# AdvancedPhotonSource/tike

Hardware: AMD Instinct MI355X
Metric: diffraction patterns/sec/GPU (256x256, 8-mode probe) (higher is better)
Workload: dtype c64; 1 GPU; c3; positions_per_gpu=10000, modes=8, detector=256, eigen_probes=1, solver=lstsq_grad, num_batch=10, chunk_positions=1000, position_correction=False, object_update=after every minibatch (batch_method wobbly_center), route=no_farplane

## Files before the change

include/tike_amd.h:

```cpp
#ifndef TIKE_AMD_H
#define TIKE_AMD_H

#ifdef __cplusplus
extern "C" {
#endif

#define TIKE_ERR_ARG 1000001
#define TIKE_ERR_UNSUPPORTED 1000002
#define TIKE_ERR_COMM 2000000
#define TIKE_COMM_ID_BYTES 128

#define TIKE_ABI_VERSION 15

const char* tike_build_id(void);

int tike_abi_version(void);

int tike_set_deterministic(int on, void* scratch, long bytes);

int tike_init(void);

int tike_patch_fwd(const void* images, void* patches, const float* positions, int nimage, int H,
                   int W, int nscan, int nrepeat, int patch_width, int padded_width,
                   void* stream);
int tike_patch_adj(void* images, const void* patches, const float* positions, int nimage, int H,
                   int W, int nscan, int nrepeat, int patch_width, int padded_width, int npatch,
                   void* stream);

int tike_conv_fwd(const void* psi, const float* scan, const void* probe, int probe_per_scan,
                  void* nearplane, int nscan, int S, int pw, int det, int H, int W, void* stream);
int tike_conv_adj(const void* nearplane, const float* scan, const void* probe,
                  int probe_per_scan, void* psi, int nscan, int S, int pw, int det, int H, int W,
                  void* stream);
int tike_conv_adj_probe(const void* nearplane, const float* scan, const void* psi,
                        void* probe_adj, int nscan, int S, int pw, int det, int H, int W,
                        void* stream);

int tike_fft2(const void* in, void* out, long ntile, int n, int inverse, float scale,
              void* stream);

int tike_fft2_supported(int n);

int tike_fft2_general(const void* in, void* out, long ntile, int n, int inverse, float scale,
                      int lines_per_group_rows, int lines_per_group_cols, void* stream);

int tike_ptycho_fwd(const void* psi, const float* scan, const void* probe, int probe_per_scan,
                    const void* eigen_probe, const float* eigen_weights, int num_eigen,
                    int eigen_modes, void* farplane, int nscan, int S, int pw, int det, int H,
                    int W, float scale, int sub_batch, void* stream);

int tike_ptycho_adj(const void* farplane, const void* probe, int probe_per_scan,
                    const float* scan, const void* psi, void* psi_adj, void* probe_adj,
                    void* objproj_work, float* acc_work, int nscan, int S, int pw, int det,
                    int H, int W, float scale, int sub_batch, void* stream);

int tike_ptycho_fwd_intensity(const void* psi, const float* scan, const void* probe,
                              int probe_per_scan, const void* unique_probe,
                              const float* eigen_weights, int num_eigen, int eigen_modes,
                              void* farplane, float* intensity, void* patches, int nscan, int S,
                              int pw, int det, int H, int W, float scale, void* stream);

int tike_ptycho_fwd_intensity_only(const void* psi, const float* scan, const void* probe,
                                   int probe_per_scan, const void* unique_probe,
                                   const float* eigen_weights, int num_eigen, int eigen_modes,
                                   void* scratch, float* intensity, int nscan, int S, int pw,
                                   int det, int H, int W, float scale, void* stream);

int tike_ptycho_fwd_gradient_scale(const void* psi, const float* scan, const void* probe,
                                   int probe_per_scan, const void* unique_probe,
                                   const float* eigen_weights, int num_eigen, int eigen_modes,
                                   void* scratch, float* intensity, void* patches,
                                   const float* data, const unsigned char* measured,
                                   float* gscale, float* costs, int nscan, int S, int pw, int det,
                                   int H, int W, float scale, int model, float unmeasured_scaling,
                                   long num_measured, void* stream);

int tike_fwd_pass1(const void* psi, const float* scan, const void* probe, int probe_per_scan,
                   const void* unique_probe, const void* eigen_probe,
                   const float* eigen_weights, int num_eigen, int eigen_modes, void* scratch,
                   void* patches, int nscan, int S, int pw, int det, int H, int W, void* stream);
int tike_fwd_gradient_scale(const void* scratch, const void* data, int data_u16,
                            const unsigned char* measured, float* gscale, float* intensity,
                            float* costs, void* farplane, int nscan, int S, int det, float scale,
                            int model, float unmeasured_scaling, long num_measured,
                            void* stream);

int tike_grad_ifft2_crop(const void* colin, const float* gscale, const float* mode_scale,
                         const unsigned char* measured, int S, void* work, void* chi,
                         long ntile, int det, int pw, float fwd_scale, float inv_scale,
                         void* stream);

int tike_fwd_grad_ifft2_pass1(const void* scratch, const void* data, int data_u16,
                              const unsigned char* measured, float* costs, void* work,
                              int nscan, int S, int det, float fwd_scale, int model,
                              float unmeasured_scaling, long num_measured, void* stream);
// ... 224 lines not shown
                         float* esum, float* work, void* stream);
int tike_eigen_dsum(const float* sums, int B, long P, float* dsum, void* stream);
int tike_eigen_weights(const float* sums, int B, long P, const float* dsum, double count,
                       float* weights_c, long weights_row, void* coefs_c, int coef_stride,
                       const float* esum, void* stream);

int tike_cgrad_direction(const float* update_planar, const void* update_complex, void* gradient,
                         void* direction, long n, int first, const float* costs, int ncost,
                         double count, double* state, double* sums, void* stream);

int tike_cgrad_line_search(int variable, const void* x, const void* d, void* xs,
                           const void* other, const float* scan, const void* data,
                           int data_u16, void* scratch, float* costs, int nscan, int chunk,
                           int S, int det, int H, int W, float fwd_scale, double count,
                           double* state, int* skip, int nslots, void* stream);

int tike_cgrad_line_search_masked(int variable, const void* x, const void* d, void* xs,
                                  const void* other, const float* scan, const void* data,
                                  int data_u16, void* scratch, float* costs, int nscan, int chunk,
                                  int S, int det, int H, int W, float fwd_scale, double count,
                                  double* state, int* skip, int nslots,
                                  const unsigned char* measured, int model, long num_measured,
                                  void* stream);

int tike_cgrad_line_search_linear(int variable, const void* x, const void* d, void* xs,
                                  const void* other, const float* scan, const void* data,
                                  int data_u16, void* far_a, int a_valid, void* far_b,
                                  float* costs_k, int nscan, int chunk, int S, int det, int H,
                                  int W, float fwd_scale, double count, double* state,
                                  int stage, double* sums, void* stream);

int tike_cgrad_line_search_linear_masked(int variable, const void* x, const void* d, void* xs,
                                         const void* other, const float* scan, const void* data,
                                         int data_u16, void* far_a, int a_valid, void* far_b,
                                         float* costs_k, int nscan, int chunk, int S, int det,
                                         int H, int W, float fwd_scale, double count,
                                         double* state, int stage, double* sums,
                                         const unsigned char* measured, int model,
                                         long num_measured, void* stream);

int tike_eigen_pixel_update1(const void* patches, const void* chi0, const void* mpu0,
                             const void* eigen0, const float* eigen_proj,
                             const float* weights_c, long weights_row, const float* norm,
                             void* update, int nscan, int pw, int chi_modes, const float* stats,
                             const float* costs, float eps, float* sums3, const void* psi,
                             const float* scan, int H, int W, void* stream);
int tike_lstsq_tail_mid(void* eigen0, const void* update, int npix, float* nacc,
                        float beta_eigen, const float* stats, int B, float eps,
                        const float* sums3, double count, int recover_psi, int recover_probe,
                        float* tail3, void* stream);
int tike_eigen_position_sums1(const void* patches, const void* chi0, const void* mpu0,
                              const void* eigen0, float* sums5, float* dsum, int nscan, int pw,
                              int chi_modes, const void* psi, const float* scan, int H, int W,
                              void* stream);
int tike_lstsq_tail_finish(const float* tail3, const float* sums3, double count, float* steps,
                           void* probe, void* combined, const void* mpu, float inv_num_batch,
                           long nprobe, float* weights, long weights_row, int S, int m,
                           const float* stats, const float* sums5, int B, int npix,
                           void* stream);

int tike_ifft2_pass2_gradients_eproj(const void* work, const void* patches, const void* probe,
                                     const void* eigen_probe, const float* eigen_weights,
                                     int num_eigen, int eigen_modes, void* objproj, void* chi0,
                                     void* m_probe_update, float mpu_scale, int nscan, int S,
                                     int det, float inv_scale, float* qtab, float* q,
                                     void* stream);
int tike_eigen_pixel_update1q(const void* patches, const void* chi0, const void* mpu0,
                              const void* eigen0, const float* q, const float* weights_c,
                              long weights_row, const float* norm, void* update, int nscan,
                              int pw, int chi_modes, const void* psi, const float* scan, int H,
                              int W, float* c0part, float* eproj_out, void* stream);
int tike_lstsq_step_stats_eigen1(const void* chi, const float* scan,
                                 const void* object_update_precond, const void* probe,
                                 const void* eigen_probe, const float* eigen_weights,
                                 int eigen_modes, const void* m_probe_update, const void* patches,
                                 const void* update, float* nacc, double count, float beta_eigen,
                                 float* stats, float* sums5, int nscan, int S, int chi_modes,
                                 int pw, int H, int W, void* stream);
int tike_lstsq_tail_solve1(void* eigen0, const void* update, int npix, const float* nacc,
                           float beta_eigen, const float* stats, const float* costs,
                           const float* sums5, int B, float eps, double count, int recover_psi,
                           int recover_probe, float* sums3, float* tail3, void* stream);

int tike_lstsq_chunk_gradients(const void* psi, const float* scan, const void* probe,
                               const void* eigen_probe, const float* eigen_weights,
                               int num_eigen, int eigen_modes, const void* data, int data_u16,
                               const unsigned char* measured, int model,
                               float unmeasured_scaling, long num_measured, void* scratch,
                               void* work, float* gscale, void* patches, float* costs,
                               void* objproj, void* chi0, void* m_probe_update,
                               float mpu_scale, float* object_acc, int nscan, int S, int det,
                               int H, int W, float fwd_scale, float inv_scale, void* stream);

int tike_lstsq_chunk_gradients_positions(
    const void* psi, const float* scan, const void* probe, const void* eigen_probe,
    const float* eigen_weights, int num_eigen, int eigen_modes, const void* data, int data_u16,
    const unsigned char* measured, int model, float unmeasured_scaling, long num_measured,
    void* scratch, void* work, float* gscale, void* patches, float* costs, void* objproj,
    void* chi0, void* m_probe_update, float mpu_scale, float* object_acc, int nscan, int S,
    int det, int H, int W, float fwd_scale, float inv_scale, const float* taps, int taps_radius,
    float* intensity_work, float* numerator, float* denominator, void* stream);

int tike_comm_unique_id(void* id);
int tike_comm_create(const void* id, int nranks, int rank, void** comm);
int tike_comm_destroy(void* comm);
int tike_comm_allreduce_sum(void* comm, void* buf, long count, int f64, void* stream);
int tike_comm_broadcast(void* comm, void* buf, long nbytes, int root, void* stream);

int tike_cluster_farthest_fill(const float* points, long n, long* owner, int num_cluster,
                               long turns);
int tike_cluster_swap_sweep(const double* dist, long n, int k, long* label, const long* best,
                            const long* order, double* regret, int* moved);

#ifdef __cplusplus
}
#endif
#endif
```

tike_amd/_lib.py:

```python
import ctypes
import os
import re

import torch

_HERE = os.path.dirname(os.path.abspath(__file__))
LIB_PATH = os.environ.get("TIKE_AMD_LIB") or os.path.join(
    _HERE, "csrc", "libtike_amd.so")
HEADER_PATH = os.path.join(os.path.dirname(_HERE), "include", "tike_amd.h")

ABI_VERSION = 15
ERR_ARG = 1000001
ERR_UNSUPPORTED = 1000002
ERR_COMM = 2000000
COMM_ID_BYTES = 128

if not os.path.isfile(LIB_PATH):
    raise ImportError(
        f"{LIB_PATH} not found: build the HIP library first "
        "(`make -C tike_amd/csrc` or `python -c 'import __graft_entry__ as g; "
        "g.build()'`). tike_amd has no CPU fallback.")

lib = ctypes.CDLL(LIB_PATH)

_p = ctypes.c_void_p
_i = ctypes.c_int
_l = ctypes.c_long
_f = ctypes.c_float
_d = ctypes.c_double

_PROTOTYPES = {
    "tike_abi_version": [],
    "tike_init": [],
    "tike_set_deterministic": [_i, _p, _l],
    "tike_patch_fwd": [_p, _p, _p, _i, _i, _i, _i, _i, _i, _i, _p],
    "tike_patch_adj": [_p, _p, _p, _i, _i, _i, _i, _i, _i, _i, _i, _p],
    "tike_conv_fwd": [_p, _p, _p, _i, _p, _i, _i, _i, _i, _i, _i, _p],
    "tike_conv_adj": [_p, _p, _p, _i, _p, _i, _i, _i, _i, _i, _i, _p],
    "tike_conv_adj_probe": [_p, _p, _p, _p, _i, _i, _i, _i, _i, _i, _p],
    "tike_fft2": [_p, _p, _l, _i, _i, _f, _p],
    "tike_fft2_supported": [_i],
    "tike_fft2_general": [_p, _p, _l, _i, _i, _f, _i, _i, _p],
    "tike_pfa_supported": [_i, _i, _i],
    "tike_pfa_fwd_gather": [_p, _p, _p, _i, _p, _p, _p, _i, _i, _p, _p, _i, _i, _i,
                            _i, _i, _i, _p],
    "tike_pfa_fwd_subtiles_supported": [_i, _i, _i],
    "tike_pfa_fwd_subtiles": [_p, _p, _p, _p, _p, _i, _i, _p, _p, _p, _i, _i,
                              _i, _i, _i, _i, _p],
    "tike_pfa_fft2": [_p, _p, _l, _i, _i, _p],
    "tike_pfa_combine_gradient": [_p, _p, _p, _p, _i, _i, _i, _f, _i, _f, _l, _i,
                                  _p],
    "tike_pfa_inv_products": [_p, _p, _p, _i, _p, _p, _p, _i, _i, _p, _p, _p, _f,
                              _i, _i, _i, _i, _f, _p],
    "tike_gen_supported": [_i, _i, _i],
    "tike_gen_fwd_rows": [_p, _p, _p, _i, _p, _p, _p, _i, _i, _p, _p, _i, _i, _i,
                          _i, _i, _i, _p],
    "tike_gen_cols_gradient": [_p, _p, _p, _p, _p, _i, _i, _i, _i, _f, _i, _f,
                               _l, _p],
    "tike_gen_inv_rows_gradients": [_p, _p, _p, _i, _p, _p, _p, _i, _i, _p, _p,
                                    _p, _f, _i, _i, _i, _i, _f, _p],
    "tike_fresnel_spect_prop": [_p, _p, _p, _l, _i, _i, _f, _f, _p],
    "tike_fft2_pass1": [_p, _p, _l, _i, _i, _p],
    "tike_fft2_pass2_inplace": [_p, _l, _i, _i, _f, _p],
    "tike_slice_step": [_p, _p, _p, _p, _i, _i, _i, _i, _i, _f, _p],
    "tike_fft2_pass2_intensity": [_p, _p, _l, _i, _i, _i, _f, _i, _p],
    "tike_fresnel_colpass": [_p, _p, _i, _p, _l, _i, _f, _p],
    "tike_ifft2_pass2_products": [_p, _p, _p, _p, _i, _p, _p, _f, _p, _i, _i, _i,
                                  _i, _i, _i, _f, _p],
    "tike_ptycho_fwd": [_p, _p, _p, _i, _p, _p, _i, _i, _p, _i, _i, _i, _i,
                        _i, _i, _f, _i, _p],
    "tike_ptycho_adj": [_p, _p, _i, _p, _p, _p, _p, _p, _p, _i, _i, _i, _i, _i,
                        _i, _f, _i, _p],
    "tike_ifft2_crop": [_p, _p, _p, _l, _i, _i, _f, _p],
    "tike_ptycho_fwd_intensity": [_p, _p, _p, _i, _p, _p, _i, _i, _p, _p, _p,
                                  _i, _i, _i, _i, _i, _i, _f, _p],
    "tike_gradient_scale": [_p, _p, _p, _p, _p, _i, _i, _i, _f, _l, _p],
    "tike_ifft2_crop_scaled": [_p, _p, _i, _p, _p, _l, _i, _i, _f, _p],
    "tike_ifft2_crop_scaled_modes": [_p, _p, _p, _p, _i, _p, _p, _l, _i, _i, _f,
                                     _p],
    "tike_poisson_steps": [_p, _p, _p, _p, _p, _i, _i, _i, _f, _f, _i, _p],
    "tike_poisson_steps_handoff": [_p, _p, _i, _p, _p, _p, _p, _p, _i, _i, _i, _f,
                                   _f, _l, _f, _f, _p],
    "tike_scale_modes": [_p, _p, _p, _l, _i, _p],
    "tike_ptycho_fwd_intensity_only": [_p, _p, _p, _i, _p, _p, _i, _i, _p, _p,
                                       _i, _i, _i, _i, _i, _i, _f, _p],
    "tike_ptycho_fwd_gradient_scale": [_p, _p, _p, _i, _p, _p, _i, _i, _p, _p,
                                       _p, _p, _p, _p, _p, _i, _i, _i, _i, _i,
                                       _i, _f, _i, _f, _l, _p],
    "tike_fwd_pass1": [_p, _p, _p, _i, _p, _p, _p, _i, _i, _p, _p, _i, _i, _i,
                       _i, _i, _i, _p],
    "tike_fwd_gradient_scale": [_p, _p, _i, _p, _p, _p, _p, _p, _i, _i, _i, _f,
                                _i, _f, _l, _p],
    "tike_grad_ifft2_pass1": [_p, _p, _p, _p, _i, _p, _l, _i, _f, _p],
    "tike_fwd_grad_ifft2_pass1": [_p, _p, _i, _p, _p, _p, _i, _i, _i, _f, _i, _f,
                                  _l, _p],
    "tike_fwd_grad_ifft2_pass1_slices": [_p, _p, _i, _p, _p, _p, _i, _i, _i, _f, _i, _f,
                                  _l, _p, _i, _p],
    "tike_ifft2_pass1_scaled": [_p, _p, _p, _p, _i, _p, _l, _i, _p],
    "tike_ifft2_pass2_gradients": [_p, _p, _p, _p, _p, _i, _i, _p, _p, _p, _f,
                                   _i, _i, _i, _f, _p],
    "tike_ifft2_pass2_gradients_scaled": [_p, _p, _p, _p, _p, _i, _i, _p, _p,
                                          _p, _f, _i, _i, _i, _f, _p, _p],
    "tike_ifft2_pass2_eigen_fits": [_i, _i, _i],
    "tike_ifft2_pass2_gradients_modes": [_p, _p, _p, _p, _p, _i, _i, _p, _p,
                                         _p, _f, _i, _i, _i, _f, _i, _i, _i, _p],
    "tike_poisson_steps_grad_ifft2_pass1": [_p, _p, _i, _p, _p, _p, _p, _p, _i,
                                            _i, _i, _f, _f, _l, _f, _f, _p],
    "tike_object_update_precond": [_p, _p, _p, _f, _p, _p, _p, _l, _p],
    "tike_lstsq_step_sums": [_p, _p, _i, _f, _p, _p],
    "tike_lstsq_step_solve": [_p, _i, _f, _p, _d, _i, _i, _p, _p],
    "tike_probe_update": [_p, _p, _p, _p, _f, _l, _p],
    "tike_eigen_weights0": [_p, _p, _i, _i, _i, _i, _p, _p],
    "tike_eigen_proj_mean": [_p, _i, _p, _l, _p, _l, _i, _p, _p],
    "tike_eigen_normalise": [_p, _p, _d, _f, _i, _p, _p, _p],
    "tike_eigen_dsum": [_p, _i, _l, _p, _p],
    "tike_eigen_weights": [_p, _i, _l, _p, _d, _p, _l, _p, _i, _p, _p],
    "tike_grad_ifft2_crop": [_p, _p, _p, _p, _i, _p, _p, _l, _i, _i, _f, _f,
                             _p],
    "tike_position_sums": [_p, _p, _i, _p, _p, _p, _i, _i, _p, _i, _p, _p, _i,
                           _i, _i, _p],
    "tike_rpie_position_sums": [_p, _p, _p, _p, _i, _p, _p, _i, _i, _p, _i, _p,
                                _p, _p, _i, _i, _i, _i, _i, _p],
    "tike_farplane_gradient": [_p, _p, _p, _p, _p, _i, _i, _i, _i, _i, _f, _l,
                               _p],
    "tike_intensity": [_p, _p, _l, _i, _l, _p],
    "tike_cost_each_pattern": [_p, _p, _p, _l, _l, _i, _p],
    "tike_objective_grad": [_p, _p, _p, _p, _l, _i, _l, _i, _p],
    "tike_lstsq_gradients": [_p, _p, _p, _p, _p, _p, _i, _i, _p, _p, _p, _p, _i,
                             _i, _i, _i, _i, _p],
    "tike_varying_probe": [_p, _p, _p, _i, _i, _p, _i, _i, _i, _p],
    "tike_scatter_patches": [_p, _p, _p, _i, _i, _i, _i, _p],
    "tike_eigen_position_sums": [_p, _p, _p, _p, _p, _i, _i, _i, _p, _i, _i,
                                 _i, _p],
    "tike_eigen_pixel_update": [_p, _p, _p, _p, _p, _i, _i, _i, _p, _p, _i, _i,
                                _i, _p],
    "tike_probe_grad": [_p, _p, _p, _p, _p, _i, _i, _i, _i, _i, _p],
    "tike_probe_preconditioner": [_p, _p, _p, _i, _i, _i, _i, _p],
    "tike_psi_preconditioner": [_p, _p, _p, _i, _i, _i, _i, _p],
    "tike_scatter_amplitudes": [_p, _p, _p, _i, _i, _i, _i, _p],
    "tike_lstsq_step_stats": [_p, _p, _p, _p, _p, _p, _p, _i, _i, _p, _p, _p,
                              _p, _i, _i, _i, _i, _i, _i, _p, _p, _p],
    "tike_eigen_pixel_update1": [_p, _p, _p, _p, _p, _p, _l, _p, _p, _i, _i, _i,
                                 _p, _p, _f, _p, _p, _p, _i, _i, _p],
    "tike_lstsq_tail_mid": [_p, _p, _i, _p, _f, _p, _i, _f, _p, _d, _i, _i, _p,
                            _p],
    "tike_eigen_position_sums1": [_p, _p, _p, _p, _p, _p, _i, _i, _i, _p, _p,
                                  _i, _i, _p],
    "tike_lstsq_tail_finish": [_p, _p, _d, _p, _p, _p, _p, _f, _l, _p, _l, _i,
                               _i, _p, _p, _i, _i, _p],
    "tike_ifft2_pass2_gradients_eproj": [_p, _p, _p, _p, _p, _i, _i, _p, _p,
                                         _p, _f, _i, _i, _i, _f, _p, _p, _p],
    "tike_eigen_pixel_update1q": [_p, _p, _p, _p, _p, _p, _l, _p, _p, _i, _i,
                                  _i, _p, _p, _i, _i, _p, _p, _p],
    "tike_lstsq_step_stats_eigen1": [_p, _p, _p, _p, _p, _p, _i, _p, _p, _p,
                                     _p, _d, _f, _p, _p, _i, _i, _i, _i, _i,
                                     _i, _p],
    "tike_lstsq_tail_solve1": [_p, _p, _i, _p, _f, _p, _p, _p, _i, _f, _d, _i,
                               _i, _p, _p, _p],
    "tike_lstsq_chunk_gradients": [_p, _p, _p, _p, _p, _i, _i, _p, _i, _p, _i,
                                   _f, _l, _p, _p, _p, _p, _p, _p, _p, _p, _f,
                                   _p, _i, _i, _i, _i, _i, _f, _f, _p],
    "tike_lstsq_chunk_gradients_positions": [
        _p, _p, _p, _p, _p, _i, _i, _p, _i, _p, _i, _f, _l, _p, _p, _p, _p, _p,
        _p, _p, _p, _f, _p, _i, _i, _i, _i, _i, _f, _f, _p, _i, _p, _p, _p, _p],
    "tike_cgrad_direction": [_p, _p, _p, _p, _l, _i, _p, _i, _d, _p, _p, _p],
    "tike_cgrad_line_search": [_i, _p, _p, _p, _p, _p, _p, _i, _p, _p, _i, _i,
                               _i, _i, _i, _i, _f, _d, _p, _p, _i, _p],
    "tike_cgrad_line_search_linear": [_i, _p, _p, _p, _p, _p, _p, _i, _p, _i, _p,
                                      _p, _i, _i, _i, _i, _i, _i, _f, _d, _p, _i,
                                      _p, _p],
    "tike_cgrad_line_search_masked": [_i, _p, _p, _p, _p, _p, _p, _i, _p, _p,
                                      _i, _i, _i, _i, _i, _i, _f, _d, _p, _p,
                                      _i, _p, _i, _l, _p],
    "tike_cgrad_line_search_linear_masked": [_i, _p, _p, _p, _p, _p, _p, _i, _p,
                                             _i, _p, _p, _i, _i, _i, _i, _i, _i,
                                             _f, _d, _p, _i, _p, _p, _i, _l, _p],
    "tike_comm_unique_id": [_p],
    "tike_comm_create": [_p, _i, _i, ctypes.POINTER(_p)],
    "tike_comm_destroy": [_p],
    "tike_comm_allreduce_sum": [_p, _p, _l, _i, _p],
    "tike_comm_broadcast": [_p, _p, _l, _i, _p],
    "tike_cluster_farthest_fill": [_p, _l, _p, _i, _l],
    "tike_cluster_swap_sweep": [_p, _l, _i, _p, _p, _p, _p, _p],
}


def build_id():
    try:
        fn = lib.tike_build_id
    except AttributeError:
        return ""
    fn.restype = ctypes.c_char_p
    fn.argtypes = []
    return fn().decode()


def declared_symbols():
    with open(HEADER_PATH) as f:
        text = f.read()
    return sorted(set(re.findall(r"^int\s+(tike_\w+)\s*\(", text, flags=re.M)))


for _name, _args in _PROTOTYPES.items():
    try:
        _fn = getattr(lib, _name)
    except AttributeError as e:
        raise ImportError(
            f"{LIB_PATH} does not export {_name}: it was built from another "
            "include/tike_amd.h; rebuild it (`make -C tike_amd/csrc`).") from e
    _fn.argtypes = _args
    _fn.restype = ctypes.c_int


def _check_abi_version():
    got = lib.tike_abi_version()
    m = re.search(r"^#define\s+TIKE_ABI_VERSION\s+(\d+)", open(HEADER_PATH).read(),
                  flags=re.M) if os.path.isfile(HEADER_PATH) else None
    if got != ABI_VERSION or (m and int(m.group(1)) != ABI_VERSION):
        raise ImportError(
            f"{LIB_PATH} reports ABI version {got}, include/tike_amd.h "
            f"{m.group(1) if m else '?'}, this binding expects {ABI_VERSION}: "
            "rebuild the library (`make -C tike_amd/csrc`).")


_check_abi_version()


def check(rc, what=""):
    if rc == 0:
        return
    if rc == ERR_ARG:
        raise ValueError(f"{what}: incompatible shapes / arguments")
    if rc == ERR_UNSUPPORTED:
        raise ValueError(f"{what}: unsupported size for the HIP path")
    if rc >= ERR_COMM:
        raise RuntimeError(f"{what}: RCCL error {rc - ERR_COMM}")
    raise RuntimeError(f"{what}: HIP error {rc}")


DETERMINISTIC = os.environ.get("TIKE_DETERMINISTIC", "0") == "1"
DETERMINISTIC_SCRATCH_MIB = int(os.environ.get("TIKE_DETERMINISTIC_MIB", "256"))
# ... 19 lines not shown
```

tike_amd/_tuning.py:

```python
import os


def _flag(name, default):
    return os.environ.get(name, "1" if default else "0") == "1"


def _int(name, default=None):
    v = os.environ.get(name)
    return int(v) if v else default


one_launch_512 = _flag("TIKE_ONE_LAUNCH_512", True)
poisson_steps_in_pass2 = _flag("TIKE_POISSON_LINEAR", True)
chunk_positions = _int("TIKE_CHUNK_POSITIONS")
eigen_sums_gather = _flag("TIKE_EIGEN_SUMS_GATHER", True)
stats_gather = _flag("TIKE_STATS_GATHER", False)
fused_tail = _flag("TIKE_FUSED_TAIL", True)
precond_chunk = _int("TIKE_PRECOND_CHUNK", 512)
multislice_slice_step = _flag("TIKE_MS_SLICE_STEP", True)
multislice_first_stored = _flag("TIKE_MS_FIRST_STORED", True)
multislice_step_back = _flag("TIKE_MS_STEP_BACK", True)
cgrad_graphs = _flag("TIKE_CGRAD_GRAPHS", False)
fwd_sub_mib = (float(os.environ["TIKE_FWD_SUB_MIB"])
               if os.environ.get("TIKE_FWD_SUB_MIB") else None)
```

tike_amd/csrc/internal.h:

```cpp
#pragma once
#include "common.h"

int tk_fft2(const cf* in, cf* out, long ntile, int n, int inverse, float scale,
            hipStream_t stream);
int tk_fft2_general(const cf* in, cf* out, long ntile, int n, int inverse, float scale,
                    int l_rows, int l_cols, hipStream_t stream);
int tk_conv_fwd(const cf* psi, const float* scan, const TkProbe& probe, cf* nearplane, int nscan,
                int S, int pw, int det, int H, int W, hipStream_t stream);
int tk_conv_adj(const cf* nearplane, const float* scan, const TkProbe& probe, cf* psi, int nscan,
                int S, int pw, int det, int H, int W, hipStream_t stream);
int tk_conv_adj_probe(const cf* nearplane, const float* scan, const cf* psi, cf* probe_adj,
                      int nscan, int S, int pw, int det, int H, int W, hipStream_t stream);

int tk_fft2_pass1(const cf* in, cf* out, long ntile, int det, bool inverse, bool keep,
                  hipStream_t stream);
int tk_ifft2_pass2_products(cf* work, const cf* psi, const float* scan, const cf* probe,
                            int probe_per_scan, cf* objproj, float* pnum, float pnum_scale,
                            cf* chi0, int out, int nscan, int S, int det, int H, int W,
                            float inv_scale, hipStream_t stream);

bool tk_deterministic();
float* tk_det_scratch(size_t bytes);

struct TkCostSink {
  float* costs;
  float* part;
  int nslots;
};
#if defined(__HIPCC__)
__device__ __forceinline__ void tk_cost_add(const TkCostSink& k, long n, int slot, float v) {
  if (k.part != nullptr)
    k.part[n * k.nslots + slot] = v;
  else
    unsafeAtomicAdd(&k.costs[n], v);
}
#endif
int tk_cost_sink(float* costs, long nscan, int nslots, hipStream_t stream, TkCostSink* sink);
int tk_cost_finish(const TkCostSink& sink, long nscan, hipStream_t stream);
int tk_ordered_sum(float* out, const float* part, long n, int nparts, bool accumulate,
                   hipStream_t stream, int out_stride = 1);
```

tike_amd/csrc/lstsq.hip:

```cpp
#include "fft_engine2.h"
#include <type_traits>

#include "internal.h"
#include "tike_amd.h"

#ifndef TK_STATS_PAIRS
#define TK_STATS_PAIRS 1
#endif
static const bool g_stats_pairs = TK_STATS_PAIRS != 0;

constexpr int TK_STRIP = 32;
#define TK_ATOMIC_ADD(p, v) unsafeAtomicAdd(p, v)

template <bool REAL_ONLY, class ValueFn, class Sink>
__device__ __forceinline__ void scatter_footprint_rows(ValueFn&& value, float fx, float fy,
                                                       int pw, int r0, int r1, Sink&& sink) {
  for (int x0 = 0; x0 < pw; x0 += blockDim.x) {
    const int xp = x0 + threadIdx.x;
    const bool active = xp < pw;
    cf uprev = mk(0.f, 0.f), uprev_last = mk(0.f, 0.f);
    constexpr int RG = 4;
    cf vv[RG], ll[RG], nv[RG], nl[RG];
    auto load_group = [&](int yb, cf (&a)[RG], cf (&b)[RG]) {
      const int xpc = active ? xp : pw - 1;
// ... 726 lines not shown
#pragma unroll
            for (int i = 0; i < 8; ++i) {
              cf t = (pc[i] * u[g + i]) * w0;
              if (REDUCE) {
                slot[(g + i) * 64] = m == 0 ? t : slot[(g + i) * 64] + t;
              } else {
                if (eig) {
#pragma unroll 1
                  for (int c = 0; c < nE; ++c)
                    t = t + (eigl[((c * probe.Sm + s) * RB + g + i) * (64 * CW) + cw * 64 + lane] *
                             u[g + i]) * wn[(c + 1) * probe.S + s];
                }
                tk_st_stream(tk_at(objproj + (long)n * P + slice0 + (g + i) * ROW, lo), t);
              }
            }
            if (!HOIST) __builtin_amdgcn_sched_barrier(0);
          }
          if (REDUCE && eig) {
#pragma unroll 1
            for (int c = 0; c < nE; ++c) {
              const float wc = wn[(c + 1) * probe.S + s];
              const cf* __restrict__ el =
                  eigl + ((c * probe.Sm + s) * RB) * (64 * CW) + cw * 64 + lane;
              if (QN && c == 0 && s == 0) {
                float q = 0.f;
#pragma unroll
                for (int yb = 0; yb < RB; ++yb) {
                  const cf e = el[yb * (64 * CW)];
                  slot[yb * 64] = slot[yb * 64] + (e * u[yb]) * wc;
                  const cf t = conjf(O[yb]) * u[yb];
                  q += t.x * e.x - t.y * e.y;
                }
                q_store(q, n);
                continue;
              }
#pragma unroll
              for (int yb = 0; yb < RB; ++yb)
                slot[yb * 64] = slot[yb * 64] + (el[yb * (64 * CW)] * u[yb]) * wc;
            }
          }
        }
      } else if (REDUCE && m == 0) {
#pragma unroll
        for (int yb = 0; yb < RB; ++yb) slot[yb * 64] = mk(0.f, 0.f);
      }
    }
    if (REDUCE) {
      __syncthreads();
#pragma unroll
      for (int q = 0; q < RB / MW; ++q) {
        const int yb = mw + MW * q;
        cf sum = slots[yb * 64];
#pragma unroll
        for (int k = 1; k < MW; ++k) sum = sum + slots[(k * RB + yb) * 64];
        if (accumulate) sum = sum + *tk_at(objproj + (long)n * P + slice0 + yb * ROW, lo);
        tk_st_stream(tk_at(objproj + (long)n * P + slice0 + yb * ROW, lo), sum);
      }
      if (NBUF == 1) __syncthreads();
    }
  }
  if (mpu != nullptr) {
#pragma unroll
    for (int m = 0; m < MPW; ++m) {
      const int s = mw + MW * m;
      if (s < S) {
#pragma unroll
        for (int yb = 0; yb < RB; ++yb) {
          if (mpu_part != nullptr) {
            const long ci = (nchunk_ - 1) - b0 / chunk;
            float* o = tk_at(mpu_part + 2 * ((ci * S + s) * P + slice0 + yb * ROW), lb);
            o[0] = acc[m][yb].x * mpu_scale;
            o[1] = acc[m][yb].y * mpu_scale;
          } else {
            float* o = tk_at(mpu + 2 * ((long)s * P + slice0 + yb * ROW), lb);
            unsafeAtomicAdd(o, acc[m][yb].x * mpu_scale);
            unsafeAtomicAdd(o + 1, acc[m][yb].y * mpu_scale);
          }
        }
      }
    }
  }
}

__global__ __launch_bounds__(256) void pass2_q_finish_kernel(const float* __restrict__ qtab,
                                                             int slots, int nscan,
                                                             float* __restrict__ q) {
  const int n = blockIdx.x * 4 + (int)(threadIdx.x >> 6), k = threadIdx.x & 63;
  if (n >= nscan) return;
  float a = k < slots ? qtab[(long)k * nscan + n] : 0.f;
  a = tk_wave_sum(a);
  if (k == 0) q[n] = a;
}

template <int N, int MW_, int MPW_>
static bool launch_pass2_qn(dim3 grid, size_t lds, hipStream_t stream, const cf* work,
                            const cf* patches, const TkProbe& pr, cf* objproj, cf* chi0,
                            float* mpu, float mpu_scale, int nscan, int S, float inv_scale,
                            int chunk, float* mpu_part, const float* mode_scale, float* qtab) {
  if constexpr (N <= 256) {
    hipLaunchKernelGGL((ifft2_pass2_gradients_kernel<N, MW_, MPW_, true, true, false, true>),
                       grid, dim3(256), lds, stream, work, patches, pr, objproj, chi0, mpu,
                       mpu_scale, nscan, S, inv_scale, chunk, mpu_part, mode_scale, 0, 0, qtab);
    return true;
  } else {
    return false;
  }
}

static int launch_pass2_gradients(const void* work, const void* patches, const void* probe,
                                  const void* eigen_probe, const float* eigen_weights,
                                  int num_eigen, int eigen_modes, void* objproj, void* chi0,
                                  void* m_probe_update, float mpu_scale, int nscan, int S,
                                  int det, float inv_scale, const float* mode_scale,
                                  hipStream_t stream, int Stot = 0, int accumulate = 0,
                                  float* qtab = nullptr, float* q = nullptr) {
  TK_CHECK_ARG(nscan >= 0 && S >= 1 && det >= 1);
  if (nscan == 0) return TK_OK;
  TK_CHECK_ARG(work && patches && (probe || !objproj));
  if (S > 8 || (det != 128 && det != 256 && det != 512)) return TK_ERR_UNSUPPORTED;
  const bool qn = q != nullptr;
  TK_CHECK_ARG(!qn || qtab);
  if (qn && (Stot != 0 || det > 256 || !objproj || !eigen_probe || !eigen_weights ||
             num_eigen < 1 || eigen_modes < 1))
    return TK_ERR_UNSUPPORTED;
  const bool grp = Stot != 0;
  if (grp && objproj && S < 2) return TK_ERR_UNSUPPORTED;
  const TkProbe pr = tk_make_probe(probe, 0, eigen_probe, eigen_weights, num_eigen, eigen_modes,
                                   grp ? Stot : S, det);
  int MW = S >= 3 ? 4 : S;
  if (det == 128 && MW == 1) MW = 2;
  auto eig_bytes = [&](int mw) {
    return sizeof(cf) * (size_t)num_eigen * eigen_modes * (det / 16) * 64 * (4 / mw);
  };
  if (objproj && eigen_weights && eigen_probe)
    while (MW < 4 && eig_bytes(MW) > 32 * 1024) MW *= 2;
  const int MPW = S > 4 ? 2 : 1;
  const int nslice = 16 * (det / (64 * (4 / MW)));
  int nchunk = (1024 + nslice - 1) / nslice;
  {
    int unit = 512, a = nslice;
    while (a % 2 == 0 && unit > 1) { a /= 2; unit /= 2; }
    if (nchunk >= unit) nchunk = nchunk / unit * unit;
  }
  int chunk = (nscan + nchunk - 1) / nchunk;
  if (chunk < 8) chunk = 8;
  nchunk = (nscan + chunk - 1) / chunk;
  const dim3 grid((unsigned)(nslice * nchunk)), block(256);
  float* mpu_part = nullptr;
  const long mpu_len = 2L * S * det * det;
  if (m_probe_update && tk_deterministic()) {
    mpu_part = tk_det_scratch(sizeof(float) * (size_t)mpu_len * nchunk);
    if (mpu_part == nullptr) return TK_ERR_ARG;
  }
  size_t eig_lds = 0;
  if (objproj && eigen_weights && eigen_probe) eig_lds = eig_bytes(MW);
  if (eig_lds > 32 * 1024) return TK_ERR_UNSUPPORTED;
#define TK_P2G(N, MW_, MPW_)                                                                 \
  do {                                                                                       \
    if (qn) {                                                                                \
      if (!launch_pass2_qn<N, MW_, MPW_>(grid, eig_lds, stream, (const cf*)work,             \
                                         (const cf*)patches, pr, (cf*)objproj, (cf*)chi0,    \
                                         (float*)m_probe_update, mpu_scale, nscan, S,        \
                                         inv_scale, chunk, mpu_part, mode_scale, qtab))      \
        return TK_ERR_UNSUPPORTED;                                                           \
    } else if (grp && !objproj)                                                              \
      hipLaunchKernelGGL((ifft2_pass2_gradients_kernel<N, MW_, MPW_, false, true, true>),    \
                         grid, block, 0,                                                     \
                         stream, (const cf*)work, (const cf*)patches, pr, (cf*)objproj,      \
                         (cf*)chi0, (float*)m_probe_update, mpu_scale, nscan, S, inv_scale,  \
                         chunk, mpu_part, mode_scale, Stot, accumulate);                     \
    else if (grp && eig_lds > 0)                                                             \
      hipLaunchKernelGGL((ifft2_pass2_gradients_kernel<N, MW_, MPW_, true, true, true>),     \
                         grid, block, eig_lds,                                               \
                         stream, (const cf*)work, (const cf*)patches, pr, (cf*)objproj,      \
                         (cf*)chi0, (float*)m_probe_update, mpu_scale, nscan, S, inv_scale,  \
                         chunk, mpu_part, mode_scale, Stot, accumulate);                     \
    else if (grp)                                                                            \
      hipLaunchKernelGGL((ifft2_pass2_gradients_kernel<N, MW_, MPW_, true, false, true>),    \
                         grid, block, 0,                                                     \
                         stream, (const cf*)work, (const cf*)patches, pr, (cf*)objproj,      \
                         (cf*)chi0, (float*)m_probe_update, mpu_scale, nscan, S, inv_scale,  \
                         chunk, mpu_part, mode_scale, Stot, accumulate);                     \
    else if (objproj && eig_lds > 0)                                                         \
      hipLaunchKernelGGL((ifft2_pass2_gradients_kernel<N, MW_, MPW_, true>), grid, block,    \
                         eig_lds,                                                            \
                         stream, (const cf*)work, (const cf*)patches, pr, (cf*)objproj,      \
                         (cf*)chi0, (float*)m_probe_update, mpu_scale, nscan, S, inv_scale,  \
                         chunk, mpu_part, mode_scale);                                       \
    else if (objproj)                                                                        \
      hipLaunchKernelGGL((ifft2_pass2_gradients_kernel<N, MW_, MPW_, true, false>), grid,    \
                         block, 0,                                                           \
                         stream, (const cf*)work, (const cf*)patches, pr, (cf*)objproj,      \
                         (cf*)chi0, (float*)m_probe_update, mpu_scale, nscan, S, inv_scale,  \
                         chunk, mpu_part, mode_scale);                                       \
    else                                                                                     \
      hipLaunchKernelGGL((ifft2_pass2_gradients_kernel<N, MW_, MPW_, false>), grid, block,   \
                         0, stream, (const cf*)work, (const cf*)patches, pr, (cf*)objproj,   \
                         (cf*)chi0, (float*)m_probe_update, mpu_scale, nscan, S, inv_scale,  \
                         chunk, mpu_part, mode_scale);                                       \
  } while (0)
#define TK_P2G_N(N)                     \
  do {                                  \
    if (MW == 1)                        \
      TK_P2G(N < 256 ? 256 : N, 1, 1);  \
    else if (MW == 2)                   \
      TK_P2G(N, 2, 1);                  \
    else if (MPW == 1)                  \
      TK_P2G(N, 4, 1);                  \
    else                                \
      TK_P2G(N, 4, 2);                  \
  } while (0)
  switch (det) {
    case 128: TK_P2G_N(128); break;
    case 256: TK_P2G_N(256); break;
    default: TK_P2G_N(512); break;
  }
#undef TK_P2G_N
#undef TK_P2G
  TK_LAUNCH_CHECK();
  if (qn) {
    hipLaunchKernelGGL(pass2_q_finish_kernel, dim3((nscan + 3) / 4), dim3(256), 0, stream,
                       qtab, det / 4, nscan, q);
    TK_LAUNCH_CHECK();
  }
  if (mpu_part != nullptr)
    return tk_ordered_sum((float*)m_probe_update, mpu_part, mpu_len, nchunk, true, stream);
  return TK_OK;
}

extern "C" int tike_ifft2_pass2_gradients(const void* work, const void* patches,
                                          const void* probe, const void* eigen_probe,
                                          const float* eigen_weights, int num_eigen,
                                          int eigen_modes, void* objproj, void* chi0,
                                          void* m_probe_update, float mpu_scale, int nscan,
                                          int S, int det, float inv_scale, void* stream) {
  TK_ENTER();
  return launch_pass2_gradients(work, patches, probe, eigen_probe, eigen_weights, num_eigen,
                                eigen_modes, objproj, chi0, m_probe_update, mpu_scale, nscan, S,
                                det, inv_scale, nullptr, (hipStream_t)stream);
}

extern "C" int tike_ifft2_pass2_gradients_scaled(const void* work, const void* patches,
                                                 const void* probe, const void* eigen_probe,
                                                 const float* eigen_weights, int num_eigen,
                                                 int eigen_modes, void* objproj, void* chi0,
                                                 void* m_probe_update, float mpu_scale,
                                                 int nscan, int S, int det, float inv_scale,
                                                 const float* mode_scale, void* stream) {
  TK_ENTER();
  TK_CHECK_ARG(nscan == 0 || mode_scale != nullptr);
  return launch_pass2_gradients(work, patches, probe, eigen_probe, eigen_weights, num_eigen,
                                eigen_modes, objproj, chi0, m_probe_update, mpu_scale, nscan, S,
                                det, inv_scale, mode_scale, (hipStream_t)stream);
}

extern "C" int tike_ifft2_pass2_gradients_eproj(const void* work, const void* patches,
                                                const void* probe, const void* eigen_probe,
                                                const float* eigen_weights, int num_eigen,
                                                int eigen_modes, void* objproj, void* chi0,
                                                void* m_probe_update, float mpu_scale,
                                                int nscan, int S, int det, float inv_scale,
                                                float* qtab, float* q, void* stream) {
  TK_ENTER();
  TK_CHECK_ARG(nscan == 0 || (qtab && q));
  return launch_pass2_gradients(work, patches, probe, eigen_probe, eigen_weights, num_eigen,
                                eigen_modes, objproj, chi0, m_probe_update, mpu_scale, nscan, S,
                                det, inv_scale, nullptr, (hipStream_t)stream, 0, 0, qtab, q);
}

extern "C" int tike_ifft2_pass2_eigen_fits(int det, int num_eigen, int eigen_modes) {
  if (det < 16 || num_eigen < 0 || eigen_modes < 0) return 0;
  return sizeof(cf) * (size_t)num_eigen * eigen_modes * (det / 16) * 64 <= 32 * 1024 ? 1 : 0;
}

extern "C" int tike_ifft2_pass2_gradients_modes(const void* work, const void* patches,
                                                const void* probe, const void* eigen_probe,
                                                const float* eigen_weights, int num_eigen,
                                                int eigen_modes, void* objproj, void* chi0,
                                                void* m_probe_update, float mpu_scale,
                                                int nscan, int S, int det, float inv_scale,
                                                int mode0, int nmodes, int accumulate,
                                                void* stream) {
  TK_ENTER();
  TK_CHECK_ARG(S >= 1 && det >= 1 && mode0 >= 0 && nmodes >= 1 && mode0 + nmodes <= S);
  TK_CHECK_ARG(nscan == 0 || (work && (probe || !objproj)));
  const long P = (long)det * det;
  const bool first = mode0 == 0;
  if (first ? eigen_modes > nmodes : false) return TK_ERR_UNSUPPORTED;
  return launch_pass2_gradients(
      (const cf*)work + mode0 * P, patches, probe ? (const cf*)probe + mode0 * P : nullptr,
      first ? eigen_probe : nullptr, eigen_weights ? eigen_weights + mode0 : nullptr,
      first ? num_eigen : (eigen_weights ? num_eigen : 0), first ? eigen_modes : 0, objproj,
      first ? chi0 : nullptr,
      m_probe_update ? (void*)((float*)m_probe_update + 2 * mode0 * P) : nullptr, mpu_scale,
      nscan, nmodes, det, inv_scale, nullptr, (hipStream_t)stream, S, accumulate);
}

template <int RW>
__global__ __launch_bounds__(256) void probe_precond_rows_kernel(
    const float* __restrict__ scan, const cf* __restrict__ psi, float* __restrict__ out,
    int nscan, int pw, int H, int W, int chunk, float* __restrict__ part) {
  typedef float tk_v4f __attribute__((ext_vector_type(4)));
  const long P = (long)pw * pw;
  const long total = (long)H * W;
  const int cols = pw < 256 ? pw : 256, ncb = pw / cols;
  const int x = ((int)blockIdx.x % ncb) * cols + (int)threadIdx.x % cols;
  const int y0 = (((int)blockIdx.x / ncb) * (256 / cols) + (int)threadIdx.x / cols) * RW;
  const int b0 = blockIdx.y * chunk;
  const int b1 = min(nscan, b0 + chunk);
  float acc[RW];
#pragma unroll
  for (int r = 0; r < RW; ++r) acc[r] = 0.f;
  bool inside = true;
  for (int b = b0; b < b1; ++b) {
    const TkCorner c = tk_corner(scan, b);
    inside = inside && c.sy >= 0 && c.sx >= 0 && c.sy + pw < H && c.sx + pw < W;
  }
  if (inside) {
    const unsigned row_bytes = (unsigned)W * (unsigned)sizeof(cf);
    const unsigned lane_off = (unsigned)y0 * row_bytes + (unsigned)x * (unsigned)sizeof(cf);
#pragma unroll 2
    for (int b = b0; b < b1; ++b) {
      const TkCorner c = tk_corner(scan, b);
      const unsigned off = (unsigned)(c.sy * W + c.sx) * (unsigned)sizeof(cf) + lane_off;
      tk_v4f t[RW + 1];
#pragma unroll
      for (int r = 0; r <= RW; ++r)
        __builtin_memcpy(&t[r], reinterpret_cast<const char*>(psi) + off + (unsigned)r * row_bytes,
                         sizeof(tk_v4f));
#pragma unroll
      for (int r = 0; r < RW; ++r) {
        cf o = mk(t[r].x * c.w00, t[r].y * c.w00);
        o.x += t[r].z * c.w01;
        o.y += t[r].w * c.w01;
        o.x += t[r + 1].x * c.w10;
        o.y += t[r + 1].y * c.w10;
        o.x += t[r + 1].z * c.w11;
        o.y += t[r + 1].w * c.w11;
        acc[r] += norm2(o);
      }
    }
  } else {
    for (int b = b0; b < b1; ++b) {
      const TkCorner c = tk_corner(scan, b);
#pragma unroll
      for (int r = 0; r < RW; ++r) {
        const int y = c.sy + y0 + r, xx = c.sx + x;
// ... 457 lines not shown
  __device__ __forceinline__ cf at(long n, long p) const {
    cf r = conjf(patches[n * P + p]) * chi0[n * XS + p] - mpu0[p];
    if (!C0)
      for (int k = 0; k < c; ++k) r = r - coefs[n * C + k] * eigen[((long)k * Sm) * P + p];
    return r;
  }
};

template <bool C0>
__global__ __launch_bounds__(256) void eigen_position_sums_kernel(const TkResidual R,
                                                                  float* __restrict__ sums,
                                                                  int nscan) {
  __shared__ float red[4];
  const cf* __restrict__ E = R.eigen + ((long)R.c * R.Sm) * R.P;
  for (int n = blockIdx.x; n < nscan; n += gridDim.x) {
    float a[5] = {0.f, 0.f, 0.f, 0.f, 0.f};
    for (long p = threadIdx.x; p < R.P; p += blockDim.x) {
      const cf e = E[p];
      const cf r = R.at<C0>(n, p);
      const cf phi = R.patches[n * R.P + p] * e;
      const cf x = R.chi0[n * R.XS + p];
      a[0] += r.x * e.x + r.y * e.y;
      a[1] += x.x * phi.x + x.y * phi.y;
      a[2] += norm2(phi);
      const cf re = r * conjf(e);
      a[3] += re.x;
      a[4] += re.y;
    }
#pragma unroll
    for (int k = 0; k < 5; ++k) {
      const float v = tk_block_sum256(a[k], red);
      if (threadIdx.x == 0) sums[(long)n * 5 + k] = v;
    }
  }
}

template <bool C0>
__global__ __launch_bounds__(256) void eigen_pixel_update_kernel(const TkResidual R,
                                                                 const float* __restrict__ pm,
                                                                 float* __restrict__ update,
                                                                 int nscan, int chunk,
                                                                 float* __restrict__ part) {
  const long p = (long)blockIdx.x * blockDim.x + threadIdx.x;
  if (p >= R.P) return;
  const int b0 = blockIdx.y * chunk;
  const int b1 = min(nscan, b0 + chunk);
  cf acc = mk(0.f, 0.f);
#pragma unroll 4
  for (int n = b0; n < b1; ++n) {
    const cf r = R.at<C0>(n, p);
    const float w = pm[n];
    acc.x += r.x * w;
    acc.y += r.y * w;
  }
  if (part != nullptr) {
    part[2 * ((long)blockIdx.y * R.P + p)] = acc.x;
    part[2 * ((long)blockIdx.y * R.P + p) + 1] = acc.y;
    return;
  }
  unsafeAtomicAdd(&update[2 * p], acc.x);
  unsafeAtomicAdd(&update[2 * p + 1], acc.y);
}

__device__ __forceinline__ cf tk_patch_pixel(const cf* __restrict__ psi, unsigned off,
                                             unsigned row_bytes, const TkCorner& c) {
  typedef float tk_v4f __attribute__((ext_vector_type(4)));
  tk_v4f u, l;
  __builtin_memcpy(&u, reinterpret_cast<const char*>(psi) + off, sizeof(u));
  __builtin_memcpy(&l, reinterpret_cast<const char*>(psi) + off + row_bytes, sizeof(l));
  cf o = mk(u.x * c.w00, u.y * c.w00);
  o.x += u.z * c.w01;
  o.y += u.w * c.w01;
  o.x += l.x * c.w10;
  o.y += l.y * c.w10;
  o.x += l.z * c.w11;
  o.y += l.w * c.w11;
  return o;
}
__device__ __forceinline__ bool tk_interior(const TkCorner& c, int pw, int H, int W) {
  return c.sy >= 0 && c.sx >= 0 && c.sy + pw < H && c.sx + pw < W && (long)H * W < (1L << 28);
}

constexpr int TK_C0_PARTS = 64;
__global__ __launch_bounds__(256) void eigen_proj_offset_kernel(const cf* __restrict__ mpu0,
                                                                const cf* __restrict__ E,
                                                                long P,
                                                                float* __restrict__ part) {
  __shared__ float red[4];
  float a = 0.f;
  for (long p = blockIdx.x * 256L + threadIdx.x; p < P; p += 256L * TK_C0_PARTS) {
    const cf m = mpu0[p], e = E[p];
    a += m.x * e.x + m.y * e.y;
  }
  a = tk_block_sum256(a, red);
  if (threadIdx.x == 0) part[blockIdx.x] = a;
}

__global__ __launch_bounds__(256) void eigen_pixel_update1_kernel(
    const TkResidual R, const float* __restrict__ eproj, const float* __restrict__ weights_c,
    long row, const float* __restrict__ norm, float inv_P, float* __restrict__ update, int nscan,
    int chunk, const float* __restrict__ stats, const float* __restrict__ costs, float eps,
    float* __restrict__ sums3, const cf* __restrict__ psi, const float* __restrict__ scan, int pw,
    int H, int W, float* __restrict__ part, const float* __restrict__ c0part,
    float* __restrict__ eproj_out) {
  float c0 = 0.f;
  if (c0part != nullptr) {
    for (int b = 0; b < TK_C0_PARTS; ++b) c0 += c0part[b];
  }
  if (blockIdx.x + 1 == gridDim.x) {
    if (blockIdx.y != 0) return;
    if (eproj_out != nullptr) {
      for (int n = threadIdx.x; n < nscan; n += 256) eproj_out[n] = eproj[n] - c0;
    }
    if (sums3 == nullptr) return;
    __shared__ float red[4];
    float a1 = 0.f, a4 = 0.f, c = 0.f;
    for (int n = threadIdx.x; n < nscan; n += 256) {
      a1 += stats[8 * n] + eps;
      a4 += stats[8 * n + 1] + eps;
      c += costs[n];
    }
    a1 = tk_block_sum256(a1, red);
    a4 = tk_block_sum256(a4, red);
    c = tk_block_sum256(c, red);
    if (threadIdx.x == 0) {
      sums3[0] = a1;
      sums3[1] = a4;
      sums3[2] = c;
    }
    return;
  }
  const long p = (long)blockIdx.x * blockDim.x + threadIdx.x;
  if (p >= R.P) return;
  const int b0 = blockIdx.y * chunk;
  const int b1 = min(nscan, b0 + chunk);
  const float inv_norm = 1.0f / norm[0];
  cf acc = mk(0.f, 0.f);
  bool gather = psi != nullptr;
  if (gather) {
    for (int n = b0; n < b1; ++n) gather = gather && tk_interior(tk_corner(scan, n), pw, H, W);
  }
  if (gather) {
    const int py = (int)(p / pw), px = (int)(p % pw);
    const unsigned row_bytes = (unsigned)W * (unsigned)sizeof(cf);
    const unsigned lane_off = (unsigned)py * row_bytes + (unsigned)px * (unsigned)sizeof(cf);
    const cf m0 = R.mpu0[p];
#pragma unroll 4
    for (int n = b0; n < b1; ++n) {
      const TkCorner c = tk_corner(scan, n);
      const cf x = R.chi0[n * R.XS + p];
      const cf o = tk_patch_pixel(
          psi, (unsigned)(c.sy * W + c.sx) * (unsigned)sizeof(cf) + lane_off, row_bytes, c);
      const cf r = conjf(o) * x - m0;
      const float w = ((eproj[n] - c0) * inv_P + weights_c[n * row]) * inv_norm;
      acc.x += r.x * w;
      acc.y += r.y * w;
    }
  } else {
#pragma unroll 4
    for (int n = b0; n < b1; ++n) {
      const cf r = R.at<true>(n, p);
      const float w = ((eproj[n] - c0) * inv_P + weights_c[n * row]) * inv_norm;
      acc.x += r.x * w;
      acc.y += r.y * w;
    }
  }
  if (part != nullptr) {
    part[2 * ((long)blockIdx.y * R.P + p)] = acc.x;
    part[2 * ((long)blockIdx.y * R.P + p) + 1] = acc.y;
    return;
  }
  unsafeAtomicAdd(&update[2 * p], acc.x);
  unsafeAtomicAdd(&update[2 * p + 1], acc.y);
}

__global__ __launch_bounds__(256) void column_sum_ordered_kernel(const float* __restrict__ table,
                                                                 int stride, int col, int n,
                                                                 float scale,
// ... 235 lines not shown
    const cf* __restrict__ chi_a = chi + ((long)n0 * chi_modes) * P;
    const cf* __restrict__ chi_b = chi + ((long)(n0 + 1) * chi_modes) * P;
    const cf* __restrict__ pat_a = patches + (long)n0 * P;
    const cf* __restrict__ pat_b = pat_a + P;
    auto tap = [](const tk_v4f u, const tk_v4f l, const TkCorner& c) {
      cf g = mk(u.x * c.w00, u.y * c.w00);
      g.x += u.z * c.w01;
      g.y += u.w * c.w01;
      g.x += l.x * c.w10;
      g.y += l.y * c.w10;
      g.x += l.z * c.w11;
      g.y += l.w * c.w11;
      return g;
    };
    auto sums = [](float* acc, const cf g, const cf o, const cf x0, const cf p0, const cf pn,
                   const cf m0) {
      const cf dOP = g * pn;
      const cf dPO = m0 * o;
      const cf OP = o * p0;
      acc[0] += norm2(dOP);
      acc[1] += norm2(dPO);
      const cf a2 = dOP * conjf(dPO);
      acc[2] += a2.x;
      acc[3] += a2.y;
      acc[4] += dOP.x * x0.x + dOP.y * x0.y;
      acc[5] += dPO.x * x0.x + dPO.y * x0.y;
      acc[6] += OP.x * x0.x + OP.y * x0.y;
      acc[7] += norm2(OP);
    };
    auto pixel = [&](const int p, const tk_v4f u0, const tk_v4f l0, const tk_v4f u1,
                     const tk_v4f l1) {
      const cf oa = pat_a[p], ob = pat_b[p];
      const cf xa = chi_a[p], xb = chi_b[p];
      const cf p0 = probe.probe[p];
      const cf m0 = mpu[p];
      const cf e1 = probe.eigen[p];
      const cf en = enew(e1, p);
      cf pa = p0 * s0, pb = p0 * s1;
      pa.x += t0 * e1.x;
      pa.y += t0 * e1.y;
      pb.x += t1 * e1.x;
      pb.y += t1 * e1.y;
      sums(a, tap(u0, l0, c0), oa, xa, p0, pa, m0);
      sums(b, tap(u1, l1, c1), ob, xb, p0, pb, m0);
      esum(ea, oa, xa, en, m0);
      esum(eb, ob, xb, en, m0);
    };
    auto taps16 = [&](const unsigned off) {
      tk_v4f t;
      __builtin_memcpy(&t, reinterpret_cast<const char*>(gobj) + off, sizeof(t));
      return t;
    };
    const int cols = pw < 256 ? pw : 256, groups = 256 / cols;
    const int rows = pw / (nsplit * groups);
    const int ybeg = (part * groups + (int)threadIdx.x / cols) * rows;
    for (int x = (int)threadIdx.x % cols; x < pw; x += 256) {
      unsigned rel = (unsigned)(ybeg * W + x);
      tk_v4f u0 = taps16((base0 + rel) * 8u), u1 = taps16((base1 + rel) * 8u);
      int p = ybeg * pw + x;
#pragma unroll 2
      for (int y = 0; y < rows; ++y) {
        rel += (unsigned)W;
        const tk_v4f l0 = taps16((base0 + rel) * 8u), l1 = taps16((base1 + rel) * 8u);
        pixel(p, u0, l0, u1, l1);
        u0 = l0;
        u1 = l1;
        p += pw;
      }
    }
#pragma unroll
    for (int k = 0; k < 8; ++k) {
      const float ta = tk_block_sum256(a[k], red);
      const float tb = tk_block_sum256(b[k], red);
      if (threadIdx.x == 0) {
        put(&stats[(long)n0 * 8 + k], ta);
        put(&stats[(long)n0 * 8 + 8 + k], tb);
      }
    }
    finish5(ea, n0);
    finish5(eb, n0 + 1);
  }
}

__global__ __launch_bounds__(256) void eigen_norm_sums1_kernel(const cf* __restrict__ E,
                                                               const cf* __restrict__ update,
                                                               int npix, float* __restrict__ nacc,
                                                               float* __restrict__ part) {
  __shared__ float red[4];
  float uu = 0.f, ee = 0.f, eu = 0.f;
  for (int i = blockIdx.x * 256 + threadIdx.x; i < npix; i += gridDim.x * 256) {
    const cf e = E[i], u = update[i];
    uu += norm2(u);
    ee += norm2(e);
    eu += e.x * u.x + e.y * u.y;
  }
  uu = tk_block_sum256(uu, red);
  ee = tk_block_sum256(ee, red);
  eu = tk_block_sum256(eu, red);
  if (threadIdx.x == 0) {
    if (part != nullptr) {
      part[3 * blockIdx.x] = uu;
      part[3 * blockIdx.x + 1] = ee;
      part[3 * blockIdx.x + 2] = eu;
    } else {
      unsafeAtomicAdd(&nacc[0], uu);
      unsafeAtomicAdd(&nacc[1], ee);
      unsafeAtomicAdd(&nacc[2], eu);
    }
  }
}

extern "C" int tike_lstsq_step_stats_eigen1(const void* chi, const float* scan,
                                            const void* object_update_precond, const void* probe,
                                            const void* eigen_probe, const float* eigen_weights,
                                            int eigen_modes, const void* m_probe_update,
                                            const void* patches, const void* update, float* nacc,
                                            double count, float beta_eigen, float* stats,
                                            float* sums5, int nscan, int S, int chi_modes,
                                            int pw, int H, int W, void* stream) {
  TK_ENTER();
  TK_CHECK_ARG(nscan >= 0 && S >= 1 && chi_modes >= 1 && pw >= 1 && H >= 1 && W >= 1 &&
               eigen_modes >= 1 && count > 0);
  TK_CHECK_ARG(probe && eigen_probe && eigen_weights && m_probe_update && update && nacc);
  const long P = (long)pw * pw;
  const long nitem = (nscan + 1) / 2;
  int nsplit = 1;
  while (nsplit < 16 && nitem * nsplit * 2 <= 8192 && P % (2048L * nsplit) == 0) nsplit *= 2;
  if (tk_deterministic()) nsplit = 1;
  const int groups = 256 / (pw < 256 ? pw : 256);
  if (!((pw % 256 == 0 || 256 % pw == 0) && pw % (nsplit * groups) == 0 &&
        (long)H * W < (1L << 28)))
    return TK_ERR_UNSUPPORTED;
  int grid = P >= 256 * 64 ? 64 : (int)((P + 255) / 256);
  float* part = nullptr;
  if (tk_deterministic()) {
    part = tk_det_scratch(sizeof(float) * 3 * (size_t)grid);
    if (part == nullptr) grid = 1;
  }
  hipLaunchKernelGGL(eigen_norm_sums1_kernel, dim3(grid), dim3(256), 0, (hipStream_t)stream,
                     (const cf*)eigen_probe, (const cf*)update, (int)P, nacc, part);
  TK_LAUNCH_CHECK();
  if (part != nullptr) {
    int rc = tk_ordered_sum(nacc, part, 3, grid, true, (hipStream_t)stream);
    if (rc) return rc;
  }
  if (nscan == 0) return TK_OK;
  TK_CHECK_ARG(chi && scan && object_update_precond && patches && stats && sums5);
  const TkProbe pr = tk_make_probe(probe, 0, eigen_probe, eigen_weights, 1, eigen_modes, S, pw,
                                   nullptr);
  if (nsplit > 1) {
    hipError_t e = hipMemsetAsync(stats, 0, sizeof(float) * 8 * (size_t)nscan, (hipStream_t)stream);
    if (e == hipSuccess)
      e = hipMemsetAsync(sums5, 0, sizeof(float) * 5 * (size_t)nscan, (hipStream_t)stream);
    if (e != hipSuccess) return (int)e;
  }
  hipLaunchKernelGGL(step_stats_eigen_pair_kernel, dim3(tk_grid(nitem * nsplit, 16)), dim3(256),
                     0, (hipStream_t)stream, (const cf*)chi, scan,
                     (const cf*)object_update_precond, pr, (const cf*)m_probe_update,
                     (const cf*)patches, (const cf*)update, (const float*)nacc,
                     (float)(1.0 / count), beta_eigen, stats, sums5, nscan, chi_modes, pw, H, W,
                     nsplit);
  TK_LAUNCH_CHECK();
  return TK_OK;
}

static TkResidual make_residual(const void* patches, const void* chi0, const void* mpu0,
                                const void* eigen, const void* coefs, int C, int Sm, int c,
                                int pw, int chi_modes) {
  TkResidual R;
  R.patches = (const cf*)patches;
  R.chi0 = (const cf*)chi0;
  R.mpu0 = (const cf*)mpu0;
  R.eigen = (const cf*)eigen;
  R.coefs = (const cf*)coefs;
  R.C = C;
  R.Sm = Sm;
  R.c = c;
  R.P = (long)pw * pw;
  R.XS = R.P * chi_modes;
  return R;
}

extern "C" int tike_eigen_position_sums(const void* patches, const void* chi0, const void* mpu0,
                                        const void* eigen_probe, const void* coefs,
                                        int num_eigen, int eigen_modes, int c, float* sums,
                                        int nscan, int pw, int chi_modes, void* stream) {
  TK_ENTER();
  TK_CHECK_ARG(nscan >= 0 && pw >= 1 && num_eigen >= 1 && c >= 0 && c < num_eigen &&
               chi_modes >= 1);
  if (nscan == 0) return TK_OK;
  TK_CHECK_ARG(patches && chi0 && mpu0 && eigen_probe && sums && (c == 0 || coefs));
  const TkResidual R = make_residual(patches, chi0, mpu0, eigen_probe, coefs, num_eigen,
                                     eigen_modes, c, pw, chi_modes);
  if (c == 0)
    hipLaunchKernelGGL(eigen_position_sums_kernel<true>, dim3(tk_grid(nscan, 16)), dim3(256), 0,
                       (hipStream_t)stream, R, sums, nscan);
  else
    hipLaunchKernelGGL(eigen_position_sums_kernel<false>, dim3(tk_grid(nscan, 16)), dim3(256),
                       0, (hipStream_t)stream, R, sums, nscan);
  TK_LAUNCH_CHECK();
  return TK_OK;
}

extern "C" int tike_eigen_pixel_update(const void* patches, const void* chi0, const void* mpu0,
                                       const void* eigen_probe, const void* coefs,
                                       int num_eigen, int eigen_modes, int c, const float* pm,
                                       void* update, int nscan, int pw, int chi_modes,
                                       void* stream) {
  TK_ENTER();
  TK_CHECK_ARG(nscan >= 0 && pw >= 1 && num_eigen >= 1 && c >= 0 && c < num_eigen &&
               chi_modes >= 1);
  if (nscan == 0) return TK_OK;
  TK_CHECK_ARG(patches && chi0 && mpu0 && eigen_probe && pm && update && (c == 0 || coefs));
  const long P = (long)pw * pw;
  float* part = nullptr;
  const int chunk = probe_chunk(nscan, 2 * P, &part);
  dim3 grid((unsigned)((P + 255) / 256), (unsigned)((nscan + chunk - 1) / chunk));
  const TkResidual R = make_residual(patches, chi0, mpu0, eigen_probe, coefs, num_eigen,
                                     eigen_modes, c, pw, chi_modes);
  if (c == 0)
    hipLaunchKernelGGL(eigen_pixel_update_kernel<true>, grid, dim3(256), 0, (hipStream_t)stream,
                       R, pm, (float*)update, nscan, chunk, part);
  else
    hipLaunchKernelGGL(eigen_pixel_update_kernel<false>, grid, dim3(256), 0,
                       (hipStream_t)stream, R, pm, (float*)update, nscan, chunk, part);
  TK_LAUNCH_CHECK();
  if (part != nullptr)
    return tk_ordered_sum((float*)update, part, 2 * P, (int)grid.y, true, (hipStream_t)stream);
  return TK_OK;
}

extern "C" int tike_eigen_pixel_update1(const void* patches, const void* chi0,
                                        const void* mpu0, const void* eigen0,
                                        const float* eigen_proj, const float* weights_c,
                                        long weights_row, const float* norm, void* update,
                                        int nscan, int pw, int chi_modes, const float* stats,
                                        const float* costs, float eps, float* sums3,
                                        const void* psi, const float* scan, int H, int W,
                                        void* stream) {
  TK_ENTER();
  TK_CHECK_ARG(nscan >= 0 && pw >= 1 && chi_modes >= 1 && weights_row >= 1);
  if (nscan == 0) {
    if (sums3) return (int)hipMemsetAsync(sums3, 0, 3 * sizeof(float), (hipStream_t)stream);
    return TK_OK;
  }
  TK_CHECK_ARG(!sums3 || (stats && costs));
  TK_CHECK_ARG(!psi || (scan && H >= 1 && W >= 1));
  TK_CHECK_ARG(patches && chi0 && mpu0 && eigen0 && eigen_proj && weights_c && norm && update);
  const long P = (long)pw * pw;
  float* part = nullptr;
  const int chunk = probe_chunk(nscan, 2 * P, &part);
  dim3 grid((unsigned)((P + 255) / 256) + 1, (unsigned)((nscan + chunk - 1) / chunk));
  const TkResidual R = make_residual(patches, chi0, mpu0, eigen0, nullptr, 1, 1, 0, pw, chi_modes);
  hipLaunchKernelGGL(eigen_pixel_update1_kernel, grid, dim3(256), 0, (hipStream_t)stream, R,
                     eigen_proj, weights_c, weights_row, norm, 1.0f / (float)P, (float*)update,
                     nscan, chunk, stats, costs, eps, sums3, (const cf*)psi, scan, pw, H, W,
                     part, nullptr, nullptr);
  TK_LAUNCH_CHECK();
  if (part != nullptr)
    return tk_ordered_sum((float*)update, part, 2 * P, (int)grid.y, true, (hipStream_t)stream);
  return TK_OK;
}

extern "C" int tike_eigen_pixel_update1q(const void* patches, const void* chi0,
                                         const void* mpu0, const void* eigen0, const float* q,
                                         const float* weights_c, long weights_row,
                                         const float* norm, void* update, int nscan, int pw,
                                         int chi_modes, const void* psi, const float* scan,
                                         int H, int W, float* c0part, float* eproj_out,
                                         void* stream) {
  TK_ENTER();
  TK_CHECK_ARG(nscan >= 0 && pw >= 1 && chi_modes >= 1 && weights_row >= 1);
  if (nscan == 0) return TK_OK;
  TK_CHECK_ARG(!psi || (scan && H >= 1 && W >= 1));
  TK_CHECK_ARG(patches && chi0 && mpu0 && eigen0 && q && weights_c && norm && update && c0part);
  const long P = (long)pw * pw;
  hipLaunchKernelGGL(eigen_proj_offset_kernel, dim3(TK_C0_PARTS), dim3(256), 0,
                     (hipStream_t)stream, (const cf*)mpu0, (const cf*)eigen0, P, c0part);
  float* part = nullptr;
  const int chunk = probe_chunk(nscan, 2 * P, &part);
  dim3 grid((unsigned)((P + 255) / 256) + 1, (unsigned)((nscan + chunk - 1) / chunk));
  const TkResidual R = make_residual(patches, chi0, mpu0, eigen0, nullptr, 1, 1, 0, pw, chi_modes);
  hipLaunchKernelGGL(eigen_pixel_update1_kernel, grid, dim3(256), 0, (hipStream_t)stream, R, q,
                     weights_c, weights_row, norm, 1.0f / (float)P, (float*)update, nscan, chunk,
                     nullptr, nullptr, 0.f, nullptr, (const cf*)psi, scan, pw, H, W, part,
                     c0part, eproj_out);
  TK_LAUNCH_CHECK();
  if (part != nullptr)
    return tk_ordered_sum((float*)update, part, 2 * P, (int)grid.y, true, (hipStream_t)stream);
  return TK_OK;
}

extern "C" int tike_eigen_position_sums1(const void* patches, const void* chi0,
                                         const void* mpu0, const void* eigen0, float* sums,
                                         float* dsum, int nscan, int pw, int chi_modes,
                                         const void* psi, const float* scan, int H, int W,
                                         void* stream) {
  TK_ENTER();
  TK_CHECK_ARG(nscan >= 0 && pw >= 1 && chi_modes >= 1);
  if (nscan == 0) return TK_OK;
  TK_CHECK_ARG(!psi || (scan && H >= 1 && W >= 1));
  TK_CHECK_ARG(patches && chi0 && mpu0 && eigen0 && sums && dsum);
  const TkResidual R = make_residual(patches, chi0, mpu0, eigen0, nullptr, 1, 1, 0, pw, chi_modes);
  const bool det = tk_deterministic();
  const int cols = pw < 256 ? pw : 256;
  const bool pairs = g_stats_pairs && psi != nullptr && nscan > 1 &&
                     (pw % 256 == 0 || 256 % pw == 0) && pw % (512 / cols) == 0 &&
                     (long)H * W < (1L << 28);
  if (pairs)
    hipLaunchKernelGGL(eigen_position_sums1_pair_kernel, dim3(tk_grid((nscan + 1) / 2, 16)),
                       dim3(512), 0, (hipStream_t)stream, R, sums, det ? nullptr : dsum, nscan,
                       (const cf*)psi, scan, pw, H, W);
  else
    hipLaunchKernelGGL(eigen_position_sums1_kernel, dim3(tk_grid(nscan, 16)), dim3(256), 0,
                       (hipStream_t)stream, R, sums, det ? nullptr : dsum, nscan, (const cf*)psi,
                       scan, pw, H, W);
  if (det)
    hipLaunchKernelGGL(column_sum_ordered_kernel, dim3(1), dim3(256), 0, (hipStream_t)stream, sums,
                       5, 2, nscan, 1.0f / (float)((long)pw * pw), dsum);
  TK_LAUNCH_CHECK();
  return TK_OK;
}

__global__ __launch_bounds__(256) void varying_probe_kernel(const TkProbe probe,
                                                            cf* __restrict__ out, long total,
                                                            long PP) {
  for (long i = blockIdx.x * (long)blockDim.x + threadIdx.x; i < total;
       i += (long)gridDim.x * blockDim.x) {
    const long pix = i % PP;
    const long ns = i / PP;
    out[i] = probe.at(ns / probe.Sm, (int)(ns % probe.Sm), pix);
  }
}

extern "C" int tike_varying_probe(const void* probe, const void* eigen_probe,
                                  const float* eigen_weights, int num_eigen, int eigen_modes,
                                  void* out, int nscan, int S, int pw, void* stream) {
  TK_ENTER();
  TK_CHECK_ARG(nscan >= 0 && S >= 1 && pw >= 1 && eigen_modes >= 1 && eigen_modes <= S);
  if (nscan == 0) return TK_OK;
  TK_CHECK_ARG(probe && eigen_weights && out && (num_eigen == 0 || eigen_probe));
  const long PP = (long)pw * pw;
  const long total = (long)nscan * eigen_modes * PP;
  hipLaunchKernelGGL(varying_probe_kernel, dim3(tk_grid((total + 255) / 256, 16)), dim3(256), 0,
                     (hipStream_t)stream,
                     tk_make_probe(probe, 0, eigen_probe, eigen_weights, num_eigen, eigen_modes,
                                   S, pw),
                     (cf*)out, total, PP);
  TK_LAUNCH_CHECK();
  return TK_OK;
}

struct TkTaps {
  float t[9];
  int r;
};

template <int RT>
__global__ __launch_bounds__(256) void position_sums_kernel(
    const cf* __restrict__ patches, const cf* __restrict__ chi, int chi_modes,
    const TkProbe probe, const TkTaps taps, float* __restrict__ num, float* __restrict__ den,
// ... 461 lines not shown
```

tike_amd/csrc/solver.hip:

```cpp
#include "internal.h"
#include "tike_amd.h"

__global__ __launch_bounds__(256) void object_update_precond_kernel(
    const float* __restrict__ acc, const cf* __restrict__ precond,
    const float* __restrict__ pmax, float alpha, cf* __restrict__ upd_sum,
    cf* __restrict__ upd_precond, float* __restrict__ combined, long npix) {
  const float am = alpha * pmax[0];
  for (long i = blockIdx.x * 256L + threadIdx.x; i < npix; i += gridDim.x * 256L) {
    const float re = acc[i], im = acc[npix + i];
    const float p = (1.0f - alpha) * precond[i].x;
    const float inv = 1.0f / sqrtf(p * p + am * am);
    if (upd_sum) upd_sum[i] = mk(re, im);
    if (upd_precond) upd_precond[i] = mk(re * inv, im * inv);
    if (combined) {
      combined[i] += re;
      combined[npix + i] += im;
    }
  }
}

extern "C" int tike_object_update_precond(const float* acc, const void* precond,
                                          const float* pmax, float alpha, void* upd_sum,
                                          void* upd_precond, float* combined, long npix,
                                          void* stream) {
  TK_ENTER();
  TK_CHECK_ARG(npix >= 0);
  if (npix == 0) return TK_OK;
  TK_CHECK_ARG(acc && precond && pmax);
  hipLaunchKernelGGL(object_update_precond_kernel, dim3(tk_grid((npix + 255) / 256, 8)),
                     dim3(256), 0, (hipStream_t)stream, acc, (const cf*)precond, pmax, alpha,
                     (cf*)upd_sum, (cf*)upd_precond, combined, npix);
  TK_LAUNCH_CHECK();
  return TK_OK;
}

__global__ __launch_bounds__(256) void step_sums_kernel(const float* __restrict__ stats,
                                                        const float* __restrict__ costs, int B,
                                                        float eps, float* __restrict__ sums) {
  __shared__ float red[4];
  float a1 = 0.f, a4 = 0.f, c = 0.f;
  for (int n = threadIdx.x; n < B; n += 256) {
    a1 += stats[8 * n] + eps;
    a4 += stats[8 * n + 1] + eps;
    if (costs) c += costs[n];
  }
  a1 = tk_block_sum256(a1, red);
  a4 = tk_block_sum256(a4, red);
  c = tk_block_sum256(c, red);
  if (threadIdx.x == 0) {
    sums[0] = a1;
    sums[1] = a4;
    sums[2] = c;
  }
}

__global__ __launch_bounds__(256) void step_solve_kernel(const float* __restrict__ stats, int B,
                                                         float eps,
                                                         const float* __restrict__ sums,
                                                         float inv_count, int recover_psi,
                                                         int recover_probe,
                                                         float* __restrict__ out) {
  __shared__ float red[4];
  const float r1 = 0.5f * sums[0] * inv_count, r4 = 0.5f * sums[1] * inv_count;
  float so = 0.f, sp = 0.f;
  for (int n = threadIdx.x; n < B; n += 256) {
    const float* s = stats + 8 * n;
    const float A1 = s[0] + eps + r1, A4 = s[1] + eps + r4;
    const float b1 = s[4], b2 = s[5];
    float x1 = 0.f, x2 = 0.f;
    if (recover_psi && recover_probe) {
      const float det = A1 * A4 - (s[2] * s[2] + s[3] * s[3]);
      x1 = -(s[2] * b2 - A4 * b1) / det;
      x2 = (A1 * b2 - s[2] * b1) / det;
    } else if (recover_psi) {
      x1 = b1 / A1;
    } else if (recover_probe) {
      x2 = b2 / A4;
    }
    so += 0.9f * fmaxf(x1, 0.f);
    sp += 0.9f * fmaxf(x2, 0.f);
  }
  so = tk_block_sum256(so, red);
  sp = tk_block_sum256(sp, red);
  if (threadIdx.x == 0) {
    out[0] = so;
    out[1] = sp;
    out[2] = so * inv_count;
    out[3] = sp * inv_count;
    out[4] = sums[2] * inv_count;
  }
}

extern "C" int tike_lstsq_step_sums(const float* stats, const float* costs, int B, float eps,
                                    float* sums, void* stream) {
  TK_ENTER();
  TK_CHECK_ARG(B >= 0 && sums && (B == 0 || stats));
  hipLaunchKernelGGL(step_sums_kernel, dim3(1), dim3(256), 0, (hipStream_t)stream, stats, costs,
                     B, eps, sums);
  TK_LAUNCH_CHECK();
  return TK_OK;
}
// ... 303 lines not shown
                       npix);
  TK_LAUNCH_CHECK();
  return TK_OK;
}

__global__ __launch_bounds__(256) void lstsq_tail_solve1_kernel(
    cf* __restrict__ E, const cf* __restrict__ update, const float* __restrict__ nacc,
    float inv_count, float beta, int npix, const float* __restrict__ stats,
    const float* __restrict__ costs, const float* __restrict__ sums5, int B, float eps,
    int recover_psi, int recover_probe, float* __restrict__ sums3, float* __restrict__ tail3) {
  if (blockIdx.x + 1 < gridDim.x) {
    const float uu = nacc[0], ee = nacc[1], eu = nacc[2];
    const float mu = sqrtf(uu * inv_count * inv_count / (float)npix);
    const float k = beta / mu * inv_count;
    const float inv = 1.0f / sqrtf((ee + 2.0f * k * eu + k * k * uu) / (float)npix);
    for (int i = blockIdx.x * 256 + threadIdx.x; i < npix; i += (gridDim.x - 1) * 256)
      E[i] = (E[i] + update[i] * k) * inv;
    return;
  }
  __shared__ float red[4];
  float a1 = 0.f, a4 = 0.f, c = 0.f, d = 0.f;
  for (int n = threadIdx.x; n < B; n += 256) {
    a1 += stats[8 * n] + eps;
    a4 += stats[8 * n + 1] + eps;
    c += costs[n];
    d += sums5[5 * n + 2] / (float)npix;
  }
  a1 = tk_block_sum256(a1, red);
  a4 = tk_block_sum256(a4, red);
  c = tk_block_sum256(c, red);
  d = tk_block_sum256(d, red);
  const float r1 = 0.5f * a1 * inv_count, r4 = 0.5f * a4 * inv_count;
  float so = 0.f, sp = 0.f;
  for (int n = threadIdx.x; n < B; n += 256) {
    const float* s = stats + 8 * n;
    const float A1 = s[0] + eps + r1, A4 = s[1] + eps + r4;
    const float b1 = s[4], b2 = s[5];
    float x1 = 0.f, x2 = 0.f;
    if (recover_psi && recover_probe) {
      const float det = A1 * A4 - (s[2] * s[2] + s[3] * s[3]);
      x1 = -(s[2] * b2 - A4 * b1) / det;
      x2 = (A1 * b2 - s[2] * b1) / det;
    } else if (recover_psi) {
      x1 = b1 / A1;
    } else if (recover_probe) {
      x2 = b2 / A4;
    }
    so += 0.9f * fmaxf(x1, 0.f);
    sp += 0.9f * fmaxf(x2, 0.f);
  }
  so = tk_block_sum256(so, red);
  sp = tk_block_sum256(sp, red);
  if (threadIdx.x == 0) {
    sums3[0] = a1;
    sums3[1] = a4;
    sums3[2] = c;
    tail3[0] = so;
    tail3[1] = sp;
    tail3[2] = d;
  }
}

extern "C" int tike_lstsq_tail_solve1(void* eigen0, const void* update, int npix,
                                      const float* nacc, float beta_eigen, const float* stats,
                                      const float* costs, const float* sums5, int B, float eps,
                                      double count, int recover_psi, int recover_probe,
                                      float* sums3, float* tail3, void* stream) {
  TK_ENTER();
  TK_CHECK_ARG(B >= 0 && count > 0 && npix >= 1 && sums3 && tail3);
  TK_CHECK_ARG(eigen0 && update && nacc && (B == 0 || (stats && costs && sums5)));
  const int grid = npix >= 256 * 64 ? 64 : (npix + 255) / 256;
  hipLaunchKernelGGL(lstsq_tail_solve1_kernel, dim3(grid + 1), dim3(256), 0, (hipStream_t)stream,
                     (cf*)eigen0, (const cf*)update, nacc, (float)(1.0 / count), beta_eigen,
                     npix, stats, costs, sums5, B, eps, recover_psi, recover_probe, sums3, tail3);
  TK_LAUNCH_CHECK();
  return TK_OK;
}

__global__ __launch_bounds__(256) void lstsq_tail_finish_kernel(
    const float* __restrict__ tail3, const float* __restrict__ sums3, float inv_count,
    float* __restrict__ steps, cf* __restrict__ probe, cf* __restrict__ combined,
    const cf* __restrict__ mpu, float inv_num_batch, long nprobe, float* __restrict__ weights,
    long row, int S, int m, const float* __restrict__ stats, const float* __restrict__ sums5,
    int B, int npix) {
  const float bp = tail3[1] * inv_count;
  const long stride = (long)gridDim.x * 256;
  const long i0 = blockIdx.x * 256L + threadIdx.x;
  if (i0 == 0) {
    steps[0] = tail3[0];
    steps[1] = tail3[1];
    steps[2] = tail3[0] * inv_count;
    steps[3] = bp;
    steps[4] = sums3[2] * inv_count;
  }
  if (probe != nullptr) {
    for (long i = i0; i < nprobe; i += stride) {
      const cf d = mpu[i] * bp;
      probe[i] = probe[i] + d;
      if (combined) combined[i] = combined[i] + d * inv_num_batch;
    }
  }
  if (weights != nullptr) {
    const float inv_P = 1.0f / (float)npix;
    const float d_mean = sums5 ? tail3[2] * inv_count : 0.f;
    for (long n = i0; n < B; n += stride) {
      weights[n * row + m] += 0.1f * stats[8 * n + 6] / stats[8 * n + 7];
      if (sums5) {
        const float* s = sums5 + 5 * n;
        weights[n * row + S + m] += (s[1] * inv_P) / (s[2] * inv_P + 0.1f * d_mean);
      }
    }
  }
}

extern "C" int tike_lstsq_tail_finish(const float* tail3, const float* sums3, double count,
                                      float* steps, void* probe, void* combined, const void* mpu,
                                      float inv_num_batch, long nprobe, float* weights,
                                      long weights_row, int S, int m, const float* stats,
                                      const float* sums5, int B, int npix, void* stream) {
  TK_ENTER();
  TK_CHECK_ARG(tail3 && sums3 && steps && count > 0 && B >= 0 && nprobe >= 0 && npix >= 0);
  TK_CHECK_ARG(!probe || mpu);
  if (B == 0) {
    weights = nullptr;
    sums5 = nullptr;
  }
  TK_CHECK_ARG(!weights || (stats && weights_row >= 1 && S >= 1 && m >= 0 && m < S));
  TK_CHECK_ARG(!sums5 || (weights && weights_row >= 2L * S && npix >= 1));
  long work = 1;
  if (probe && nprobe > work) work = nprobe;
  if (weights && B > work) work = B;
  hipLaunchKernelGGL(lstsq_tail_finish_kernel, dim3(tk_grid((work + 255) / 256, 8)), dim3(256), 0,
                     (hipStream_t)stream, tail3, sums3, (float)(1.0 / count), steps, (cf*)probe,
                     (cf*)combined, (const cf*)mpu, inv_num_batch, nprobe, weights, weights_row,
                     S, m, stats, sums5, B, npix);
  TK_LAUNCH_CHECK();
  return TK_OK;
}

static int chunk_body(
    const void* psi, const float* scan, const void* probe, const void* eigen_probe,
    const float* eigen_weights, int num_eigen, int eigen_modes, const void* data, int data_u16,
    const unsigned char* measured, int model, float unmeasured_scaling, long num_measured,
    void* scratch, void* work, float* gscale, void* patches, float* costs, void* objproj,
    void* chi0, void* m_probe_update, float mpu_scale, float* object_acc, int nscan, int S,
    int det, int H, int W, float fwd_scale, float inv_scale, void* stream) {
  if (!((det == 128 && S <= 8) || (det == 256 && S <= 8) || (det == 512 && S <= 4)))
    return TK_ERR_UNSUPPORTED;
  TK_CHECK_ARG(gscale || det == 256);
  if (det == 128) {
    if (data_u16 || (eigen_weights && eigen_modes > 0)) return TK_ERR_UNSUPPORTED;
    float* inten = gscale + (size_t)nscan * det * det;
    int rc = tike_ptycho_fwd_intensity(psi, scan, probe, 0, nullptr, eigen_weights, num_eigen,
                                       eigen_modes, scratch, inten, patches, nscan, S, det, det,
                                       H, W, fwd_scale, stream);
    if (rc) return rc;
    rc = tike_gradient_scale(inten, (const float*)data, measured, gscale, costs, nscan, det,
                             model, unmeasured_scaling, num_measured, stream);
    if (rc) return rc;
    rc = tike_ifft2_pass1_scaled(scratch, gscale, nullptr, nullptr, S, work, (long)nscan * S, det,
                                 stream);
    if (rc) return rc;
    rc = tike_ifft2_pass2_gradients(work, patches, probe, eigen_probe, eigen_weights, num_eigen,
                                    eigen_modes, objproj, chi0, m_probe_update, mpu_scale, nscan,
                                    S, det, inv_scale, stream);
    if (rc) return rc;
    if (object_acc) rc = tike_scatter_patches(objproj, scan, object_acc, nscan, det, H, W, stream);
    return rc;
  }
  int rc = tike_fwd_pass1(psi, scan, probe, 0, nullptr, eigen_probe, eigen_weights, num_eigen,
                          eigen_modes, scratch, patches, nscan, S, det, det, H, W, stream);
  if (rc) return rc;
  if (det == 256) {
    rc = tike_fwd_grad_ifft2_pass1(scratch, data, data_u16, measured, costs, work, nscan, S, det,
                                   fwd_scale, model, unmeasured_scaling, num_measured, stream);
  } else {
    rc = tike_fwd_gradient_scale(scratch, data, data_u16, measured, gscale, nullptr, costs,
                                 nullptr, nscan, S, det, fwd_scale, model, unmeasured_scaling,
                                 num_measured, stream);
    if (rc) return rc;
    rc = tike_grad_ifft2_pass1(scratch, gscale, nullptr, nullptr, S, work, (long)nscan * S, det,
                               fwd_scale, stream);
  }
  if (rc) return rc;
  rc = tike_ifft2_pass2_gradients(work, patches, probe, eigen_probe, eigen_weights, num_eigen,
                                  eigen_modes, objproj, chi0, m_probe_update, mpu_scale, nscan,
                                  S, det, inv_scale, stream);
  if (rc) return rc;
  if (object_acc) rc = tike_scatter_patches(objproj, scan, object_acc, nscan, det, H, W, stream);
  return rc;
}

extern "C" int tike_lstsq_chunk_gradients(
    const void* psi, const float* scan, const void* probe, const void* eigen_probe,
    const float* eigen_weights, int num_eigen, int eigen_modes, const void* data, int data_u16,
    const unsigned char* measured, int model, float unmeasured_scaling, long num_measured,
    void* scratch, void* work, float* gscale, void* patches, float* costs, void* objproj,
    void* chi0, void* m_probe_update, float mpu_scale, float* object_acc, int nscan, int S,
    int det, int H, int W, float fwd_scale, float inv_scale, void* stream) {
  TK_ENTER();
  TK_CHECK_ARG(nscan >= 0 && S >= 1 && H >= 1 && W >= 1);
  if (nscan == 0) return TK_OK;
  TK_CHECK_ARG(psi && scan && probe && data && scratch && work && patches);
  TK_CHECK_ARG(scratch != work && (object_acc == nullptr) == (objproj == nullptr));
  return chunk_body(psi, scan, probe, eigen_probe, eigen_weights, num_eigen, eigen_modes, data,
                    data_u16, measured, model, unmeasured_scaling, num_measured, scratch, work,
                    gscale, patches, costs, objproj, chi0, m_probe_update, mpu_scale, object_acc,
                    nscan, S, det, H, W, fwd_scale, inv_scale, stream);
}

extern "C" int tike_lstsq_chunk_gradients_positions(
    const void* psi, const float* scan, const void* probe, const void* eigen_probe,
    const float* eigen_weights, int num_eigen, int eigen_modes, const void* data, int data_u16,
    const unsigned char* measured, int model, float unmeasured_scaling, long num_measured,
    void* scratch, void* work, float* gscale, void* patches, float* costs, void* objproj,
    void* chi0, void* m_probe_update, float mpu_scale, float* object_acc, int nscan, int S,
    int det, int H, int W, float fwd_scale, float inv_scale, const float* taps, int taps_radius,
    float* intensity_work, float* numerator, float* denominator, void* stream) {
  TK_ENTER();
  TK_CHECK_ARG(nscan >= 0 && S >= 1 && H >= 1 && W >= 1);
// ... 19 lines not shown
```

tike_amd/ptycho/solvers/_plan.py:

```python
from dataclasses import dataclass
from types import SimpleNamespace

import torch

from ... import _arrays as A
from ..._lib import check, lib

MODELS = {"gaussian": 0, "poisson": 1}


def algorithmic_bytes(name, n, S, det, pw, C, depth=1):
    T = 8 * S * det * det
    Tw = 8 * S * pw * det
    P = 8 * pw * pw
    D = 4 * det * det
    box = 8 * (pw + 1) * (pw + 1)
    table = {
        "tike_fwd_pass1": n * (T + 2 * P + 8) + (S + C) * P,
        "tike_fwd_gradient_scale": n * (T + 2 * D),
        "tike_fwd_pass1:cost_only": n * (T + P + 8) + (S + C) * P,
        "tike_fwd_gradient_scale:cost_only": n * (T + D + 4),
        "tike_ptycho_fwd_gradient_scale":
        n * (T + P + 2 * D + 8) + (S + C) * P,
        "tike_ptycho_fwd_intensity": n * (T + P + D + 8) + (S + C) * P,
        "tike_ptycho_fwd_intensity_only": n * (T + P + D + 8) + (S + C) * P,
        "tike_ifft2_crop_scaled": n * (T + S * P + D),
        "tike_grad_ifft2_crop": n * (T + S * P + D),
        "tike_grad_ifft2_pass1": n * (2 * T + D),
        "tike_fwd_grad_ifft2_pass1": n * (2 * T + D),
        "tike_poisson_steps_grad_ifft2_pass1": n * (3 * T + 2 * D),
        "tike_ifft2_pass2_gradients_scaled": n * (T + 3 * P) + S * P,
        "tike_ifft2_pass2_gradients": n * (T + 3 * P) + S * P,
        "tike_ifft2_pass2_gradients_modes": n * (T + 3 * P) + S * P,
        "tike_lstsq_chunk_gradients":
        (n * (T + 2 * P + 8) + (S + C) * P)
        + (n * (2 * T + D) if det == 256 else n * (T + 2 * D) + n * (2 * T + D))
        + (n * (T + 2 * P) + S * P) + n * (P + box),
        "tike_gradient_scale": n * 3 * D,
        "tike_farplane_gradient": n * (2 * T + D + 4),
        "tike_ifft2_crop": n * (T + S * P),
        "tike_lstsq_gradients": n * (S * P + 2 * P),
        "tike_scatter_patches": n * (P + box),
        "tike_lstsq_step_stats": n * (3 * P + 32),
        "tike_gen_fwd_rows": n * (Tw + 2 * P + 8) + (S + C) * P,
        "tike_gen_cols_gradient": n * (2 * Tw + D),
        "tike_gen_inv_rows_gradients": n * (Tw + 3 * P) + S * P,
        "tike_pfa_fwd_gather": n * (T + 2 * P + 8) + (S + C) * P,
        "tike_pfa_fft2": n * 2 * T,
        "tike_pfa_combine_gradient": n * (2 * T + D),
        "tike_pfa_inv_products": n * (T + 3 * P) + S * P,
        "tike_fwd_pass1:no_patches": n * (T + P + 8) + (S + C) * P,
        "tike_fwd_pass1:incident": n * (2 * T + P + 8),
        "tike_fresnel_colpass": n * 2 * T + D * 2,
        "tike_fft2_pass2_inplace": n * 2 * T,
        "tike_fft2_pass2_intensity": n * (T + D),
        "tike_fwd_grad_ifft2_pass1_slices": n * (T + D + depth * T),
        "tike_ifft2_pass2_products": n * (T + 3 * P) + S * P,
        "tike_ifft2_pass2_products:incident": n * (2 * T + 2 * P),
    }
    return table.get(name, 0)


@dataclass(frozen=True)
class GradientPlan:
    det: int
    pw: int
    S: int
    model: int
    poisson: bool
    dominant: int
    all_modes: bool
    masked: bool
    route: str
    fused: bool
    general: bool
    pfa: bool
    pos_major: bool
    no_farplane: bool
    split_kept: bool
    one_launch: bool
    steps_in_pass2: bool
    chunk: int
    launches: tuple
    groups: tuple = ()
    plain: bool = False

    def bytes(self, entry, n, C=0):
        return algorithmic_bytes(entry, n, self.S, self.det, self.pw, C)

    @staticmethod
    def for_(op, S, pw, det, exitwave_options, mask_u8, eigen_modes=0,
             num_eigen=0, plain=False):
        from . import lstsq as L
        eo = exitwave_options
        unmeasured = float(eo.unmeasured_pixels_scaling)
        from ... import _lib
        key = (_lib.DETERMINISTIC, S, pw, det, eo.noise_model,
               None if plain else eo.step_length_usemodes,
               mask_u8 is not None, True if plain else unmeasured == 1.0,
               tuple(L.POSITION_MAJOR_SIZES), tuple(L.NO_FARPLANE_SIZES),
               tuple(L.SPLIT_FORWARD_SIZES), tuple(L.ONE_LAUNCH_GRADIENT_SIZES),
               L.POISSON_FROM_HANDOFF, L.POISSON_STEPS_IN_PASS2,
               L.GENERAL_FUSED, L.PFA_ROUTE, L.GENERAL_MIN_DETECTOR,
               L.CHUNK_POSITIONS_OVERRIDE,
               L.mode_groups(S, pw, det, eigen_modes),
               bool(lib.tike_ifft2_pass2_eigen_fits(det, num_eigen,
                                                    eigen_modes)),
               bool(plain))
        cache = op.__dict__.setdefault("_tike_amd_plans", {})
        if key not in cache:
            cache[key] = GradientPlan._build(S, pw, det, eo, mask_u8, unmeasured,
                                             L, eigen_modes, key[-2], key[-1])
        return cache[key]

    @staticmethod
    def _build(S, pw, det, eo, mask_u8, unmeasured, L, eigen_modes=0,
               eigen_fits=True, plain=False):
        poisson = eo.noise_model == "poisson" and not plain
        dominant = int(poisson and eo.step_length_usemodes == "dominant_mode")
        all_modes = poisson and not dominant
        pos_major = det in L.POSITION_MAJOR_SIZES
        fused = L.fused_gradients(S, pw, det)
        groups = () if fused or poisson else L.mode_groups(S, pw, det,
                                                           eigen_modes)
        fused = (fused or bool(groups)) and eigen_fits
        groups = groups if fused else ()
# ... 266 lines not shown
        if self.fused:
            check(
                lib.tike_ifft2_pass1_scaled(
                    A.ptr(b.far), A.ptr(b.gscale),
                    A.ptr(b.steps) if self.poisson else None,
                    A.ptr(c.mask_u8) if self.poisson else None, S,
                    A.ptr(b.mid), n * S, det, st), "scaled inverse pass 1")
        elif self.poisson:
            check(
                lib.tike_ifft2_crop_scaled_modes(
                    A.ptr(b.far), A.ptr(b.gscale), A.ptr(b.steps),
                    A.ptr(c.mask_u8), S, A.ptr(b.mid), A.ptr(b.chi), n * S,
                    det, pw, c.inv_scale, st), "scaled ifft2 + crop (poisson)")
        else:
            check(
                lib.tike_ifft2_crop_scaled(A.ptr(b.far), A.ptr(b.gscale), S,
                                           A.ptr(b.mid), A.ptr(b.chi), n * S,
                                           det, pw, c.inv_scale, st),
                "scaled ifft2 + crop")

    def _forward_unfused(self, c, k):
        b, S, det, pw = c.buf, self.S, self.det, self.pw
        n, st, d = k.n, c.st, k.data_f32()
        c.op.fwd_device(c.probe, k.scan, c.psi, c.eigen_probe, k.w,
                        out=b.far[:n])
        if self.poisson:
            check(lib.tike_intensity(A.ptr(b.far), A.ptr(b.inten), n, S,
                                     det * det, st), "intensity")
            check(
                lib.tike_poisson_steps(
                    A.ptr(b.far), A.ptr(b.inten), A.ptr(d), A.ptr(c.mask_u8),
                    A.ptr(b.steps), n, S, det, c.step_start, c.step_weight,
                    self.dominant, st), "poisson step lengths")
        check(
            lib.tike_farplane_gradient(
                A.ptr(b.far), A.ptr(d), A.ptr(c.mask_u8), None, A.ptr(k.costs),
                n, S, det, self.model, 1, c.unmeasured, c.nmeasured, st),
            "farplane gradient")
        if self.poisson:
            check(
                lib.tike_scale_modes(A.ptr(b.far), A.ptr(b.steps),
                                     A.ptr(c.mask_u8), n * S, det, st),
                "poisson step scaling")
        check(
            lib.tike_ifft2_crop(A.ptr(b.far), A.ptr(b.mid), A.ptr(b.chi), n * S,
                                det, pw, c.inv_scale, st), "ifft2 + crop")

    def gradients(self, c, k):
        b, S, det, pw = c.buf, self.S, self.det, self.pw
        n, st = k.n, c.st
        objproj = (A.ptr(b.objproj) if getattr(c, "want_objproj",
                                               c.recover_psi) else None)
        chi0 = A.ptr(k.chi0) if c.need_chi0 and k.chi0 is not None else None
        if self.pfa:
            check(
                lib.tike_pfa_inv_products(
                    A.ptr(b.far), A.ptr(k.patches), A.ptr(c.probe), 0, None,
                    A.ptr(c.ep), A.ptr(k.w), c.C, c.Sm, objproj, chi0,
                    A.ptr(c.m_probe_update), 1.0 / c.num_batch, n, S, pw, det,
                    c.inv_scale, st), "prime-factor inverse products")
        elif self.general:
            check(
                lib.tike_gen_inv_rows_gradients(
                    A.ptr(b.mid), A.ptr(k.patches), A.ptr(c.probe), 0, None,
                    A.ptr(c.ep), A.ptr(k.w), c.C, c.Sm, objproj, chi0,
                    A.ptr(c.m_probe_update), 1.0 / c.num_batch, n, S, pw, det,
                    c.inv_scale, st), "general inverse rows + gradients")
        elif self.fused:
            p2 = (A.ptr(b.far if self.split_kept else b.mid), A.ptr(k.patches),
                  A.ptr(c.probe), A.ptr(c.ep), A.ptr(k.w), c.C, c.Sm, objproj,
                  chi0, A.ptr(c.m_probe_update), 1.0 / c.num_batch, n, S, det,
                  c.inv_scale)
            if self.groups:
                for first, count in self.groups:
                    check(lib.tike_ifft2_pass2_gradients_modes(
                        *p2, first, count, int(first > 0), st),
                        "inverse pass 2 + gradients (a group of modes)")
            elif self.steps_in_pass2:
                check(lib.tike_ifft2_pass2_gradients_scaled(
                    *p2, A.ptr(b.steps), st),
                    "inverse pass 2 + gradients (x poisson steps)")
            elif k.q is not None:
                check(lib.tike_ifft2_pass2_gradients_eproj(
                    *p2, A.ptr(b.qtab), A.ptr(k.q), st),
                    "inverse pass 2 + gradients + eigen projection")
            else:
                check(lib.tike_ifft2_pass2_gradients(*p2, st),
                      "inverse pass 2 + gradients")
        else:
            check(
                lib.tike_lstsq_gradients(
                    A.ptr(b.chi), A.ptr(k.scan), A.ptr(c.psi), A.ptr(c.probe),
                    A.ptr(c.ep), A.ptr(k.w), c.C, c.Sm,
                    None,
                    A.ptr(k.patches), A.ptr(c.m_probe_update), objproj, n, S,
                    pw, c.H, c.W, st), "probe gradient + object projection")
```

tike_amd/ptycho/solvers/lstsq.py:

```python
import logging
from types import SimpleNamespace

import numpy as np
import torch

from ... import _arrays as A
from ... import _tuning
from ... import linalg
from ... import opt
from ... import random as trandom
from ..._lib import check, lib
from ...operators.propagation import fft_scales
from ..position import gaussian_derivative_taps
from ._plan import GradientPlan

logger = logging.getLogger(__name__)

_MODELS = {"gaussian": 0, "poisson": 1}


class _Workspace:

    def __init__(self):
        self.buffers = {}

    def get(self, name, shape, dtype, device):
        n = int(np.prod(shape))
        buf = self.buffers.get(name)
        if (buf is None or buf.numel() < n or buf.dtype != dtype
                or buf.device != device):
            buf = torch.empty(n, dtype=dtype, device=device)
            self.buffers[name] = buf
        return buf[:n].view(*shape)


def _workspace(op):
    ws = getattr(op, "_tike_amd_workspace", None)
    if ws is None:
        ws = op._tike_amd_workspace = _Workspace()
    return ws


POSITION_MAJOR_SIZES = (128, 256, 512)
NO_FARPLANE_SIZES = (256,)
SPLIT_FORWARD_SIZES = (256, 512)
"""Detector sizes served by the position-major forward kernel
(tike_ptycho_fwd_intensity) and the gradient-scaled inverse."""


ONE_LAUNCH_GRADIENT_SIZES = (256, 512)
"""Detector sizes whose forward column pass, gradient factor and inverse pass
1 are one launch (tike_fwd_grad_ifft2_pass1; 512^2 since round 5); A/B runs
and tests shorten it to fall back to the two launches."""
if not _tuning.one_launch_512:
    ONE_LAUNCH_GRADIENT_SIZES = (256,)

POISSON_FROM_HANDOFF = True
"""Per-mode poisson step lengths at 256^2 / 512^2 from the forward hand-off
(tike_poisson_steps_handoff) instead of from a stored far plane; tests set
this to False to compare the two pipelines."""

POISSON_STEPS_IN_PASS2 = _tuning.poisson_steps_in_pass2
"""Every pixel measured, 256^2: the second sweep of the per-mode poisson step
lengths and the gradient pass in one launch, the steps applied by pass 2
(tike_poisson_steps_grad_ifft2_pass1)."""

CHUNK_POSITIONS_OVERRIDE = _tuning.chunk_positions
"""Tests set this to force small kernel chunks (several per minibatch);
TIKE_CHUNK_POSITIONS does the same for A/B runs of the bench."""


GENERAL_FUSED = True
"""Shapes outside `fused_gradients` (probe window < detector, more than 8
modes, detector sizes with factors 3 / 5 / 7 ...) run the three general
launches of csrc/general.hip (tike_gen_*; gaussian model) instead of the
unfused round-1 kernels; tests set this to False to compare the two."""


GENERAL_MIN_DETECTOR = 1 << 30
"""Detector sizes below this (and without a prime-factor decomposition) keep
the unfused kernels.  Late in round 6 that is every size: with 384, 768 and
1024 -- the sizes where the LDS line engine's three launches were 10 ... 17 %
ahead -- on the prime-factor kernels, what is left to it loses to the unfused
kernels on the mixed-radix transforms or ties with them (300^2 x 1 ... 8 modes
-43 ... -6 %, 400^2 +-0, 500^2 x 4 +7 %, 600^2 x 2 -12 %, 720^2 x 4 -15 %, 1000^2
x 1 ... 4 -3 ... -25 %; with an eigen probe -14 ... +7 %:
profiles/r06_experiments.md section 17).  The launches stay in the tree and
in the tests (`GENERAL_FUSED = "always"`); 256 restores round 6's first rule."""

# ... 66 lines not shown
    return (getattr(comm, "minibatch", None), lo, hi, comm.size)


def mask_info(exitwave_options, det=None):
    mask = exitwave_options.measured_pixels
    if det is not None and tuple(mask.shape) != (det, det):
        raise ValueError(
            f"measured_pixels shape {tuple(mask.shape)} does not match the "
            f"detector ({det}, {det})")
    key = (id(mask), tuple(mask.shape))
    cached = exitwave_options.__dict__.get("_mask_info")
    if cached is None or cached[0] != key:
        m = mask if A.is_device(mask) else A.to_device(
            np.asarray(mask, dtype=bool))
        n = int(m.sum().item())
        info = (n, None if n == m.numel() else m.to(torch.uint8).contiguous())
        cached = (key, info)
        exitwave_options.__dict__["_mask_info"] = cached
    return cached[1]


def lstsq_grad(parameters, data, batches, comm, *, op, epoch):
    scan = parameters.scan
    psi = parameters.psi
    probe = parameters.probe
    algorithm_options = parameters.algorithm_options
    eigen_weights = parameters.eigen_weights
    eigen_probe = parameters.eigen_probe
    exitwave_options = parameters.exitwave_options
    object_options = parameters.object_options
    probe_options = parameters.probe_options
    position_options = parameters.position_options
    if exitwave_options.noise_model not in _MODELS:
        raise ValueError(
            f"unknown noise model {exitwave_options.noise_model!r}")
    recover_probe = (probe_options is not None
                     and epoch >= probe_options.update_start)
    recover_psi = object_options is not None
    num_batch = algorithm_options.num_batch
    compact = algorithm_options.batch_method == "compact"
    order = (range(num_batch) if compact else
             trandom.randomizer_np.permutation(num_batch))
    if hasattr(data, "hint"):
        data.hint([_lo_hi(batches[b]) for b in order])

    dev = psi.device
    H, W = psi.shape[-2:]
    object_combined = (torch.zeros((2, H, W), dtype=torch.float32, device=dev)
                       if recover_psi and compact else None)
    probe_combined_update = torch.zeros_like(probe)
    steps = torch.zeros((num_batch, 5), dtype=torch.float32, device=dev)
    pmax = None
    if recover_psi:
        pmax = torch.amax(object_options.preconditioner.real).reshape(
            1).contiguous()
    beta_object, beta_probe = [], []
    position_terms = None
    if position_options is not None:
        position_terms = (torch.zeros_like(scan), torch.zeros_like(scan))
    packed = PACKED_TAIL and (eigen_probe is None
                              or eigen_probe.shape[-4] == 1)
    eigen_norms = None
    if (packed and recover_probe and eigen_weights is not None
            and eigen_probe is not None):
        eigen_norms = torch.stack([
            torch.square(eigen_weights[_lo_hi(b)[0]:_lo_hi(b)[1], 1, 0]).sum()
            for b in batches
        ]).to(torch.float32).contiguous()
        if comm.collective:
            comm.Allreduce(eigen_norms)

    want_q = bool(FUSED_TAIL and eigen_norms is not None and recover_psi
                  and not comm.collective and not STATS_PATCH_RECOMPUTE)

    for batch_index in order:
        lo, hi = _lo_hi(batches[batch_index])
        comm.minibatch = int(batch_index)
        g = _get_nearplane_gradients(
            data, psi, scan, probe, eigen_probe, eigen_weights, lo, hi, comm,
            num_batch=num_batch, exitwave_options=exitwave_options, op=op,
            recover_psi=recover_psi, recover_probe=recover_probe,
            position_terms=position_terms, want_q=want_q)

        object_update_precond = None
        if recover_psi:
            object_update_precond = _precondition_object_update(
                g["object_acc"], object_options.preconditioner, pmax=pmax,
                combined=object_combined)
        if packed:
            bbeta_object, bbeta_probe = _packed_tail(
                g, psi, scan, probe, eigen_probe, eigen_weights,
                object_update_precond, lo, hi, comm, op=op,
                num_batch=num_batch, recover_psi=recover_psi,
                recover_probe=recover_probe,
                norm=None if eigen_norms is None else
                eigen_norms[batch_index:batch_index + 1],
                steps_row=steps[batch_index],
                probe_combined_update=probe_combined_update)
        else:
            stats = _step_stats(g, psi, scan, probe, eigen_probe,
                                object_update_precond, lo, hi, op=op)

            if recover_probe and eigen_weights is not None:
                eigen_probe, eigen_weights = _update_nearplane(
                    g, stats, probe, eigen_probe, eigen_weights, lo, hi, comm,
                    num_batch=num_batch)

            bbeta_object, bbeta_probe, _ = _solve_steps(
                stats, g["costs"], g["count"], comm, pw=probe.shape[-1],
                recover_psi=recover_psi, recover_probe=recover_probe,
                out=steps[batch_index])

        if recover_psi:
            if not compact:
                dpsi = bbeta_object * object_update_precond
                if object_options.use_adaptive_moment:
                    dpsi, object_options.v, object_options.m = opt.momentum(
                        g=dpsi, v=object_options.v, m=object_options.m,
                        vdecay=object_options.vdecay,
                        mdecay=object_options.mdecay)
                psi = psi + dpsi
            beta_object.append(bbeta_object)

        if recover_probe:
            if not packed:
                check(
                    lib.tike_probe_update(A.ptr(probe),
                                          A.ptr(probe_combined_update),
                                          A.ptr(g["m_probe_update"]),
                                          A.ptr(bbeta_probe), 1.0 / num_batch,
                                          probe.numel(), A.stream_ptr()),
                    "probe update")
            beta_probe.append(bbeta_probe)

    batch_cost = steps[:, 4]
    if position_options is not None:
        scan = _update_position(scan, position_options, *position_terms, comm,
                                epoch=epoch)

    algorithm_options.costs.append([float(batch_cost.mean().item())])
    if (eigen_weights is not None and eigen_weights.shape[1] > 1
            and not np.isfinite(algorithm_options.costs[-1][0])):
        nonzero = torch.stack([
            (eigen_weights[int(idx[0]):int(idx[0]) + len(idx), 1:, 0]
             != 0).sum(dim=0).to(torch.float32) if len(idx) else torch.zeros(
                 eigen_weights.shape[1] - 1, device=psi.device)
            for idx in batches
        ])
        if comm.collective:
            comm.Allreduce(nonzero)
        if bool((nonzero == 0).any().item()):
            raise ValueError("eigen_probe weights cannot all be zero?")

    if recover_psi and compact:
        object_update_precond = _precondition_object_update(
            object_combined, object_options.preconditioner, pmax=pmax)
        bo = torch.mean(torch.stack(beta_object))
        dpsi = bo * object_update_precond
        psi = psi + dpsi
        if object_options.use_adaptive_moment:
            dpsi, object_options.v, object_options.m = _momentum_checked(
                g=dpsi, v=object_options.v, m=object_options.m,
                mdecay=object_options.mdecay,
                errors=[float(x[0]) for x in algorithm_options.costs[-3:]],
                beta=bo, memory_length=3)
            weight = object_options.preconditioner
            weight = weight / (0.1 * weight.real.max() + weight)
            psi = psi + weight * dpsi

    if recover_probe and probe_options.use_adaptive_moment:
        bp = torch.mean(torch.stack(beta_probe))
        dprobe = probe_combined_update
        if probe_options.v is None:
            probe_options.v = torch.zeros((3, *dprobe.shape),
                                          dtype=dprobe.dtype,
                                          device=dprobe.device)
        if probe_options.m is None:
            probe_options.m = torch.zeros_like(dprobe)
        mode = 0
        (d, probe_options.v[..., mode, :, :],
         probe_options.m[..., mode, :, :]) = _momentum_checked(
             g=dprobe[..., mode, :, :], v=probe_options.v[..., mode, :, :],
             m=probe_options.m[..., mode, :, :], mdecay=probe_options.mdecay,
             errors=[float(x[0]) for x in algorithm_options.costs[-3:]],
             beta=bp, memory_length=3)
        probe[..., mode, :, :] = probe[..., mode, :, :] + d

    parameters.scan = scan
    parameters.psi = psi
    parameters.probe = probe
    parameters.eigen_weights = eigen_weights
    parameters.eigen_probe = eigen_probe
    return parameters


EIGEN_PATCH_RECOMPUTE = True
"""The eigen pixel update of the packed tail gathers the object patches from
psi (L2) instead of streaming the stored ones (HBM): 0.186 -> 0.160 ms per 1000
positions at 256^2.  (With two 16-byte tap loads per pixel the position sums
lost by it, 0.215 -> 0.221 ms; see EIGEN_SUMS_RECOMPUTE.)"""

EIGEN_SUMS_RECOMPUTE = _tuning.eigen_sums_gather
"""The position sums gather too, through the two-positions-per-workgroup row
walk of tike_eigen_position_sums1 (one 16-byte tap load per pixel and
position, E_0 and the probe update loaded once per pair): 0.215 -> 0.176 ms
per 1000 positions at 256^2."""

STATS_PATCH_RECOMPUTE = _tuning.stats_gather
"""The step statistics gather O_n from the object with the two 16-byte tap
loads they already issue for the preconditioned update (same offsets)."""

FUSED_TAIL = _tuning.fused_tail
"""One rank, one eigen probe, the fused pass 2 at 128^2 / 256^2: pass 2 leaves
the per-position part of the eigen projection, the eigen update runs before
the step statistics, and the statistics and the eigen position sums are one
pass over chi_n,0 and the patches (tike_lstsq_step_stats_eigen1)."""

PACKED_TAIL = True
"""Tests set this to False to run the staged tail (one entry per step of the
reference's _update_nearplane / _precondition_nearplane_gradients)."""


def _lo_hi(batch):
    lo = int(batch[0]) if len(batch) else 0
    return lo, lo + len(batch)


def _eigen_args(eigen_probe, weights):
    if weights is None:
        return None, None, 0, 0
    C = Sm = 0
    if eigen_probe is not None:
        C, Sm = eigen_probe.shape[-4], eigen_probe.shape[-3]
    assert weights.shape[1] == C + 1, (weights.shape, C)
    return eigen_probe, weights, C, Sm


def _once(make):
    box = []

    def get():
        if not box:
            box.append(make())
        return box[0]

    return get


def _get_nearplane_gradients(data, psi, scan, probe, eigen_probe,
                             eigen_weights, lo, hi, comm, *, num_batch,
                             exitwave_options, op, recover_psi, recover_probe,
                             position_terms=None, need_chi0=True,
                             want_q=False, plain=False,
                             all_mode_position_terms=None):
    dev = psi.device
    B = hi - lo
    S, pw = probe.shape[-3], probe.shape[-1]
    det = op.detector_shape
    H, W = psi.shape[-2:]
    if exitwave_options.noise_model not in _MODELS:
        raise ValueError(
            f"unknown noise model {exitwave_options.noise_model!r}")
    nmeasured, mask_u8 = mask_info(exitwave_options, det)
    fwd_scale, inv_scale = fft_scales(det, op.norm)

    w_old = None if eigen_weights is None else eigen_weights[lo:hi]
    ep, _, C, Sm = _eigen_args(eigen_probe, w_old)
    plan = GradientPlan.for_(op, S, pw, det, exitwave_options, mask_u8,
                             eigen_modes=Sm, num_eigen=C, plain=plain)

    n_obj = 2 * H * W if recover_psi else 0
    n_prb = 2 * probe.numel() if recover_probe else 0
    grads = torch.zeros(n_obj + n_prb, dtype=torch.float32, device=dev)
    obj_acc = grads[:n_obj].view(2, H, W) if recover_psi else None
    m_probe_update = (torch.view_as_complex(
        grads[n_obj:].view(*probe.shape, 2)) if recover_probe else None)
    probe_sum = None
    early = bool(comm.collective and recover_psi and recover_probe)
    buf = plan.buffers(
        _workspace(op), B, dev, varying=Sm if w_old is not None else 0,
        want_patches=bool((recover_probe and eigen_weights is not None)
                          or position_terms))
    if position_terms:
        taps, taps_r = gaussian_derivative_taps(sigma=0.333)
    q = None
    if (want_q and recover_psi and recover_probe and w_old is not None
            and buf.patches is not None and need_chi0
            and plan.eigen_q(C, Sm, H, W)):
        q = _workspace(op).get("eigen_q", (max(B, 1),), torch.float32, dev)
        buf.qtab = _workspace(op).get("eigen_qtab", (min(plan.chunk, max(B, 1)),
                                                     det // 4),
                                      torch.float32, dev)
    c = SimpleNamespace(
        op=op, data=data, psi=psi, probe=probe, ep=ep, eigen_probe=eigen_probe,
        C=C, Sm=Sm, H=H, W=W, st=A.stream_ptr(), fwd_scale=fwd_scale,
        inv_scale=inv_scale, nmeasured=nmeasured, mask_u8=mask_u8,
        unmeasured=(1.0 if plain else
                    float(exitwave_options.unmeasured_pixels_scaling)),
        step_start=float(exitwave_options.step_length_start),
        step_weight=float(exitwave_options.step_length_weight), buf=buf,
        m_probe_update=m_probe_update, num_batch=num_batch,
        recover_psi=recover_psi, need_chi0=need_chi0,
        want_objproj=bool(recover_psi or all_mode_position_terms))
    chunk = plan.chunk
    for clo in range(lo, hi, chunk):
        chi_hi = min(hi, clo + chunk)
        n, blo = chi_hi - clo, clo - lo
        rows = slice(blo, blo + n)
        k = SimpleNamespace(
            n=n, scan=scan[clo:chi_hi], data=data[clo:chi_hi],
            w=None if w_old is None else w_old[rows], uq=None,
            costs=buf.costs[rows],
            patches=None if buf.patches is None else buf.patches[rows],
            chi0=None if buf.chi0 is None else buf.chi0[rows],
            q=None if q is None else q[rows])
        k.data_f32 = _once(lambda a=clo, b=chi_hi: A.data_f32(data, a, b))
        if k.w is not None and Sm > 0 and buf.unique is not None and (
                not plan.no_farplane):
            k.uq = buf.unique[:n]
            check(
                lib.tike_varying_probe(A.ptr(probe), A.ptr(ep), A.ptr(k.w), C,
                                       Sm, A.ptr(k.uq), n, S, pw, c.st),
                "varying probe")
        plan.forward(c, k)
        plan.gradients(c, k)
        stored_chi0 = plan.fused or plan.general
        if position_terms:
            chi_m, chi_modes = ((k.chi0, 1) if stored_chi0 else (buf.chi, S))
            check(
                lib.tike_position_sums(
                    A.ptr(k.patches), A.ptr(chi_m), chi_modes, A.ptr(probe),
                    A.ptr(ep), A.ptr(k.w), C, Sm, taps.ctypes.data, taps_r,
                    A.ptr(position_terms[0][clo:chi_hi]),
                    A.ptr(position_terms[1][clo:chi_hi]), n, S, pw, c.st),
                "position shift sums")
        if all_mode_position_terms:
            all_mode_position_sums(
                op, buf.objproj[:n], psi, k.scan, probe, ep, k.w,
                all_mode_position_terms[0][clo:chi_hi],
                all_mode_position_terms[1][clo:chi_hi])
        if chi_hi == hi and early:
            probe_sum = comm.Allreduce_start(grads[n_obj:])
        if recover_psi:
            check(
                lib.tike_scatter_patches(A.ptr(buf.objproj), A.ptr(k.scan),
                                         A.ptr(obj_acc), n, pw, H, W, c.st),
                "object scatter")
        if not buf.single_chunk and not stored_chi0:
            buf.chi0[rows] = buf.chi[:n, 0, 0]

    if comm.collective and grads.numel():
        if early:
            if probe_sum is None:
                probe_sum = comm.Allreduce_start(grads[n_obj:])
            comm.Allreduce(grads[:n_obj])
            probe_sum.wait()
        else:
            comm.Allreduce(grads)
    count = global_count(comm, op, lo, hi)
    if recover_probe and not (plan.fused or plan.general):
        m_probe_update = m_probe_update / num_batch
    return dict(chi0=buf.chi if buf.single_chunk else buf.chi0[:B],
                chi_modes=S if buf.single_chunk else 1, w_old=w_old,
                patches=None if buf.patches is None else buf.patches[:B],
                object_acc=obj_acc, m_probe_update=m_probe_update,
                costs=buf.costs[:B], count=count, local_count=B,
                q=None if q is None else q[:B])


def all_mode_position_sums(op, objproj, psi, scan, probe, eigen_probe, weights,
                           numerator, denominator, *, per_scan=False):
    n = objproj.shape[0]
    S, pw = probe.shape[-3], probe.shape[-1]
    taps, taps_r = gaussian_derivative_taps(sigma=0.333)
    ep, w, C, Sm = _eigen_args(eigen_probe, weights)
    work = _workspace(op).get("probe_intensity", (pw, pw), torch.float32,
                              psi.device)
    check(
        lib.tike_rpie_position_sums(
            A.ptr(objproj), A.ptr(psi[0]), A.ptr(scan), A.ptr(probe),
            int(per_scan), A.ptr(ep), A.ptr(w), C, Sm, taps.ctypes.data,
            taps_r, A.ptr(work), A.ptr(numerator), A.ptr(denominator), n, S,
            pw, psi.shape[-2], psi.shape[-1], A.stream_ptr()),
        "position shift sums (all modes)")


def positions_allowed_flag(scan, psi_shape, pw):
    corner = torch.floor(scan)
    room = torch.tensor([psi_shape[-2] - pw - 1, psi_shape[-1] - pw - 1],
                        dtype=scan.dtype, device=scan.device)
    ok = ((corner >= 1) & (corner <= room)).all()
    return (~ok).to(torch.float32)


def object_upd_sum(g):
    acc = g["object_acc"]
    return None if acc is None else torch.complex(acc[0], acc[1])[None]


def _precondition_object_update(object_acc, psi_update_denominator,
                                alpha=0.05, *, pmax=None, combined=None):
    H, W = object_acc.shape[-2:]
    if pmax is None:
        pmax = torch.amax(psi_update_denominator.real).reshape(1).contiguous()
    out = torch.empty((1, H, W), dtype=torch.complex64,
                      device=object_acc.device)
    check(
        lib.tike_object_update_precond(A.ptr(object_acc),
                                       A.ptr(psi_update_denominator),
                                       A.ptr(pmax), alpha, None, A.ptr(out),
                                       A.ptr(combined), H * W, A.stream_ptr()),
        "preconditioned object update")
    return out


def _step_stats(g, psi, scan, probe, eigen_probe, object_update_precond, lo,
                hi, *, op):
    B = hi - lo
    dev = psi.device
    S, pw = probe.shape[-3], probe.shape[-1]
    stats = _workspace(op).get("stats", (max(B, 1), 8), torch.float32, dev)
    ep, w_old, C, Sm = _eigen_args(eigen_probe, g["w_old"])
    eigen0 = eproj = None
    if (ep is not None and C >= 1 and Sm >= 1 and g["patches"] is not None
            and g["m_probe_update"] is not None):
        eigen0 = ep[0, 0, 0]
        eproj = _workspace(op).get("eigen_proj", (max(B, 1),), torch.float32,
                                   dev)
    g["eigen_proj"] = None if eproj is None else eproj[:B]
    check(
        lib.tike_lstsq_step_stats(
            A.ptr(g["chi0"]), A.ptr(scan[lo:hi]), A.ptr(psi),
            A.ptr(object_update_precond), A.ptr(probe), A.ptr(ep),
            A.ptr(w_old), C, Sm, None, A.ptr(g["m_probe_update"]),
            None if (STATS_PATCH_RECOMPUTE and psi.shape[0] == 1
                     and object_update_precond is not None) else
            A.ptr(g["patches"]), A.ptr(stats), B,
            S, g["chi_modes"], pw, psi.shape[-2], psi.shape[-1],
            A.ptr(eigen0), A.ptr(eproj), A.stream_ptr()),
        "step-size statistics")
    return stats[:B]


def _packed_tail(g, psi, scan, probe, eigen_probe, eigen_weights,
                 object_update_precond, lo, hi, comm, *, op, num_batch,
                 recover_psi, recover_probe, norm, steps_row,
                 probe_combined_update):
    B = hi - lo
    dev = psi.device
    st = A.stream_ptr()
    S, pw = probe.shape[-3], probe.shape[-1]
    P = pw * pw
    count = float(g["count"])
    ws = _workspace(op)
    eig = recover_probe and eigen_weights is not None
    C = Sm = 0
    if eig and eigen_probe is not None:
        C, Sm = eigen_probe.shape[-4], eigen_probe.shape[-3]
        assert eigen_weights.shape[-2] == C + 1 and C == 1
    mpu = g["m_probe_update"]
    one = (eig and C == 1 and Sm >= 1 and g["patches"] is not None
           and mpu is not None and norm is not None)
    assert one or C == 0, "packed tail: eigen probe without its operands"
    small = ws.get("tail_small", (4 + 2 * P + 8,), torch.float32, dev)
    small.zero_()
    sums3 = small[:3]
    update = small[4:4 + 2 * P]
    nacc = small[4 + 2 * P:4 + 2 * P + 4]
    tail3 = small[4 + 2 * P + 4:4 + 2 * P + 7]
    if (one and g.get("q") is not None and not comm.collective
            and object_update_precond is not None and psi.shape[0] == 1):
        return _fused_tail(g, psi, scan, probe, eigen_probe, eigen_weights,
                           object_update_precond, lo, hi, op=op,
                           num_batch=num_batch, recover_psi=recover_psi,
                           recover_probe=recover_probe, norm=norm,
                           steps_row=steps_row,
                           probe_combined_update=probe_combined_update,
                           sums3=sums3, update=update, nacc=nacc, tail3=tail3)
    stats = _step_stats(g, psi, scan, probe, eigen_probe,
                        object_update_precond, lo, hi, op=op)
    eps_total = float(np.float32(np.float32(1e-9) / P) * P)
    E = w_rows = sums5 = None
    row = 0
    if eig:
        w_rows = eigen_weights[lo:hi]
        row = w_rows.shape[-2] * w_rows.shape[-1]
    gpsi = A.ptr(psi[0]) if EIGEN_PATCH_RECOMPUTE and psi.shape[0] == 1 else None
    if one:
        E = eigen_probe[0, 0, 0]
        check(
            lib.tike_eigen_pixel_update1(
                A.ptr(g["patches"]), A.ptr(g["chi0"]), A.ptr(mpu[0, 0, 0]),
                A.ptr(E), A.ptr(g["eigen_proj"]), w_rows[:, 1, 0].data_ptr(),
                row, A.ptr(norm), A.ptr(update), B, pw, g["chi_modes"],
                A.ptr(stats), A.ptr(g["costs"]), eps_total, A.ptr(sums3),
                gpsi, A.ptr(scan[lo:hi]), psi.shape[-2], psi.shape[-1], st),
            "eigen pixel update")
    else:
        check(
            lib.tike_lstsq_step_sums(A.ptr(stats), A.ptr(g["costs"]), B,
                                     eps_total, A.ptr(sums3), st),
            "step-size sums")
    if comm.collective:
        comm.Allreduce(small[:4 + 2 * P] if one else small[:4])
    beta_eigen = min(0.1, 1.0 / num_batch)
    check(
        lib.tike_lstsq_tail_mid(A.ptr(E), A.ptr(update), P, A.ptr(nacc),
                                beta_eigen, A.ptr(stats), B, eps_total,
                                A.ptr(sums3), count, int(recover_psi),
                                int(recover_probe), A.ptr(tail3), st),
        "step solve")
    if one:
        sums5 = ws.get("eigen_sums5", (max(B, 1), 5), torch.float32, dev)
        check(
            lib.tike_eigen_position_sums1(
                A.ptr(g["patches"]), A.ptr(g["chi0"]), A.ptr(mpu[0, 0, 0]),
                A.ptr(E), A.ptr(sums5), tail3[2:].data_ptr(), B, pw,
                g["chi_modes"], gpsi if EIGEN_SUMS_RECOMPUTE else None,
                A.ptr(scan[lo:hi]), psi.shape[-2], psi.shape[-1], st),
            "eigen position sums")
    if comm.collective:
        comm.Allreduce(tail3)
    check(
        lib.tike_lstsq_tail_finish(
            A.ptr(tail3), A.ptr(sums3), count, A.ptr(steps_row),
            A.ptr(probe) if recover_probe else None,
            A.ptr(probe_combined_update) if recover_probe else None,
            A.ptr(mpu), 1.0 / num_batch, probe.numel(),
            None if w_rows is None else w_rows.data_ptr(), row, S, 0,
            A.ptr(stats), A.ptr(sums5), B, P, st), "minibatch tail")
    return (steps_row[2] if recover_psi else None,
            steps_row[3] if recover_probe else None)


def _fused_tail(g, psi, scan, probe, eigen_probe, eigen_weights,
                object_update_precond, lo, hi, *, op, num_batch, recover_psi,
                recover_probe, norm, steps_row, probe_combined_update, sums3,
                update, nacc, tail3):
    B = hi - lo
    dev = psi.device
    st = A.stream_ptr()
    S, pw = probe.shape[-3], probe.shape[-1]
    P = pw * pw
    H, W = psi.shape[-2:]
    count = float(g["count"])
    ws = _workspace(op)
    mpu = g["m_probe_update"]
    Sm = eigen_probe.shape[-3]
    w_rows = eigen_weights[lo:hi]
    row = w_rows.shape[-2] * w_rows.shape[-1]
    E = eigen_probe[0, 0, 0]
    eps_total = float(np.float32(np.float32(1e-9) / P) * P)
    stats = ws.get("stats", (max(B, 1), 8), torch.float32, dev)
    sums5 = ws.get("eigen_sums5", (max(B, 1), 5), torch.float32, dev)
    eproj = ws.get("eigen_proj", (max(B, 1),), torch.float32, dev)
    c0part = ws.get("eigen_c0part", (64,), torch.float32, dev)
    g["eigen_proj"] = eproj[:B]
    gpsi = A.ptr(psi[0]) if EIGEN_PATCH_RECOMPUTE else None
    scan_b = A.ptr(scan[lo:hi])
    check(
        lib.tike_eigen_pixel_update1q(
            A.ptr(g["patches"]), A.ptr(g["chi0"]), A.ptr(mpu[0, 0, 0]),
            A.ptr(E), A.ptr(g["q"]), w_rows[:, 1, 0].data_ptr(), row,
            A.ptr(norm), A.ptr(update), B, pw, g["chi_modes"], gpsi, scan_b,
            H, W, A.ptr(c0part), A.ptr(eproj), st),
        "eigen pixel update")
    beta_eigen = min(0.1, 1.0 / num_batch)
    check(
        lib.tike_lstsq_step_stats_eigen1(
            A.ptr(g["chi0"]), scan_b, A.ptr(object_update_precond),
            A.ptr(probe), A.ptr(eigen_probe), A.ptr(g["w_old"]), Sm,
            A.ptr(mpu), A.ptr(g["patches"]), A.ptr(update), A.ptr(nacc), count,
            beta_eigen, A.ptr(stats), A.ptr(sums5), B, S, g["chi_modes"], pw,
            H, W, st),
        "step-size statistics + eigen position sums")
    check(
        lib.tike_lstsq_tail_solve1(
            A.ptr(E), A.ptr(update), P, A.ptr(nacc), beta_eigen, A.ptr(stats),
            A.ptr(g["costs"]), A.ptr(sums5), B, eps_total, count,
            int(recover_psi), int(recover_probe), A.ptr(sums3), A.ptr(tail3),
            st), "eigen probe + step solve")
    check(
        lib.tike_lstsq_tail_finish(
            A.ptr(tail3), A.ptr(sums3), count, A.ptr(steps_row),
            A.ptr(probe) if recover_probe else None,
            A.ptr(probe_combined_update) if recover_probe else None,
            A.ptr(mpu), 1.0 / num_batch, probe.numel(), w_rows.data_ptr(), row,
            S, 0, A.ptr(stats), A.ptr(sums5), B, P, st), "minibatch tail")
    g["stats"] = stats[:B]
    g["sums5"] = sums5[:B]
    return (steps_row[2] if recover_psi else None,
            steps_row[3] if recover_probe else None)


def _solve_steps(stats, costs, count, comm, *, pw, recover_psi, recover_probe,
                 out=None):
    dev = stats.device
    B = stats.shape[0]
    st = A.stream_ptr()
    eps_total = float(np.float32(np.float32(1e-9) / (pw * pw)) * (pw * pw))
    if out is None:
        out = torch.zeros(5, dtype=torch.float32, device=dev)
    sums = torch.empty(3, dtype=torch.float32, device=dev)
    check(
        lib.tike_lstsq_step_sums(A.ptr(stats), A.ptr(costs), B, eps_total,
                                 A.ptr(sums), st), "step-size sums")
    if comm.collective:
        comm.Allreduce(sums)
    check(
        lib.tike_lstsq_step_solve(A.ptr(stats), B, eps_total, A.ptr(sums),
                                  float(count), int(recover_psi),
                                  int(recover_probe), A.ptr(out), st),
        "step-size solve")
    if comm.collective:
        comm.Allreduce(out[:2])
        out[2:4] = out[:2] / count
    return (out[2] if recover_psi else None,
            out[3] if recover_probe else None, out[4])


def _update_nearplane(g, stats, probe, eigen_probe, eigen_weights, lo, hi,
                      comm, *, num_batch):
    m = 0
    dev = probe.device
    count = float(g["count"])
    B = hi - lo
    st = A.stream_ptr()
    Cw, S = eigen_weights.shape[-2] - 1, eigen_weights.shape[-1]
    row = (Cw + 1) * S
    w_rows = eigen_weights[lo:hi]
    norms = torch.empty(max(Cw, 1), dtype=torch.float32, device=dev)
    check(
        lib.tike_eigen_weights0(A.ptr(w_rows), A.ptr(stats), B, Cw, S, m,
                                A.ptr(norms), st), "eigen weights (shared)")
    if Cw < 1 or eigen_probe is None:
        return eigen_probe, eigen_weights
    if m >= eigen_probe.shape[-3]:
        return eigen_probe, eigen_weights
    assert eigen_weights.shape[-2] == eigen_probe.shape[-4] + 1
    if comm.collective:
        comm.Allreduce(norms)
    chi0, patches = g["chi0"], g["patches"]
    mpu0 = g["m_probe_update"][0, 0, m]
    C, Sm, pw = eigen_probe.shape[-4], eigen_probe.shape[-3], probe.shape[-1]
    P = pw * pw
    beta = min(0.1, 1.0 / num_batch)
    sums = torch.empty((max(B, 1), 5), dtype=torch.float32, device=dev)
    coefs = torch.zeros((max(B, 1), C), dtype=torch.complex64, device=dev)
    pm = torch.empty(max(B, 1), dtype=torch.float32, device=dev)
    small = torch.empty(2, dtype=torch.float32, device=dev)
    nwork = torch.empty(4, dtype=torch.float32, device=dev)
    ep = eigen_probe

    def position_sums(c):
        check(
            lib.tike_eigen_position_sums(A.ptr(patches), A.ptr(chi0),
                                         A.ptr(mpu0), A.ptr(ep), A.ptr(coefs),
                                         C, Sm, c, A.ptr(sums), B, pw,
                                         g["chi_modes"], st),
            "eigen position sums")

    for c in range(1, C + 1):
        w_c = w_rows[:, c, m]
        if c == 1 and g.get("eigen_proj") is not None:
            first, stride = g["eigen_proj"], 1
        else:
            position_sums(c - 1)
            first, stride = sums, 5
        check(
            lib.tike_eigen_proj_mean(A.ptr(first), stride, w_c.data_ptr(), row,
                                     norms[c - 1:].data_ptr(), P, B,
# ... 75 lines not shown
```

Baseline: 219,000 patterns/s.

## Fuse minibatch tail kernels: prepare, precond+norms, and psi update into finish

```diff
diff --git a/include/tike_amd.h b/include/tike_amd.h
--- a/include/tike_amd.h
+++ b/include/tike_amd.h
@@ -10,7 +10,7 @@
 #define TIKE_ERR_COMM 2000000
 #define TIKE_COMM_ID_BYTES 128
 
-#define TIKE_ABI_VERSION 15
+#define TIKE_ABI_VERSION 16
 
 const char* tike_build_id(void);
 
@@ -401,6 +401,34 @@
                            const float* sums5, int B, float eps, double count, int recover_psi,
                            int recover_probe, float* sums3, float* tail3, void* stream);
 
+int tike_lstsq_tail_prepare1(const float* qtab, int slots, int nscan, float* q, const void* mpu0,
+                             const void* eigen0, int npix, float* c0part, float* arena,
+                             long arena_len, void* stream);
+int tike_eigen_pixel_update1p(const void* patches, const void* chi0, const void* mpu0,
+                              const void* eigen0, const float* q, const float* weights_c,
+                              long weights_row, const float* norm, void* update, int nscan,
+                              int pw, int chi_modes, const void* psi, const float* scan, int H,
+                              int W, const float* c0part, float* eproj_out, void* stream);
+int tike_object_precond_eigen_norms1(const float* acc, const void* precond, const float* pmax,
+                                     float alpha, void* upd_precond, float* combined,
+                                     long npix_obj, const void* eigen0, const void* update,
+                                     int npix, float* nacc, void* stream);
+int tike_lstsq_step_stats_eigen1f(const void* chi, const float* scan,
+                                  const void* object_update_precond, const void* probe,
+                                  const void* eigen_probe, const float* eigen_weights,
+                                  int eigen_modes, const void* m_probe_update,
+                                  const void* patches, const void* update, float* nacc,
+                                  double count, float beta_eigen, float* stats, float* sums5,
+                                  int nscan, int S, int chi_modes, int pw, int H, int W,
+                                  int flags, void* stream);
+int tike_lstsq_tail_finish_psi(const float* tail3, const float* sums3, double count,
+                               float* steps, void* probe, void* combined, const void* mpu,
+                               float inv_num_batch, long nprobe, float* weights,
+                               long weights_row, int S, int m, const float* stats,
+                               const float* sums5, int B, int npix, const void* psi,
+                               const void* object_update, void* psi_next, long npsi,
+                               void* stream);
+
 int tike_lstsq_chunk_gradients(const void* psi, const float* scan, const void* probe,
                                const void* eigen_probe, const float* eigen_weights,
                                int num_eigen, int eigen_modes, const void* data, int data_u16,
diff --git a/tike_amd/_lib.py b/tike_amd/_lib.py
--- a/tike_amd/_lib.py
+++ b/tike_amd/_lib.py
@@ -9,7 +9,7 @@
     _HERE, "csrc", "libtike_amd.so")
 HEADER_PATH = os.path.join(os.path.dirname(_HERE), "include", "tike_amd.h")
 
-ABI_VERSION = 15
+ABI_VERSION = 16
 ERR_ARG = 1000001
 ERR_UNSUPPORTED = 1000002
 ERR_COMM = 2000000
@@ -157,6 +157,16 @@
                                      _i, _p],
     "tike_lstsq_tail_solve1": [_p, _p, _i, _p, _f, _p, _p, _p, _i, _f, _d, _i,
                                _i, _p, _p, _p],
+    "tike_lstsq_tail_prepare1": [_p, _i, _i, _p, _p, _p, _i, _p, _p, _l, _p],
+    "tike_eigen_pixel_update1p": [_p, _p, _p, _p, _p, _p, _l, _p, _p, _i, _i,
+                                  _i, _p, _p, _i, _i, _p, _p, _p],
+    "tike_object_precond_eigen_norms1": [_p, _p, _p, _f, _p, _p, _l, _p, _p, _i,
+                                         _p, _p],
+    "tike_lstsq_step_stats_eigen1f": [_p, _p, _p, _p, _p, _p, _i, _p, _p, _p,
+                                      _p, _d, _f, _p, _p, _i, _i, _i, _i, _i,
+                                      _i, _i, _p],
+    "tike_lstsq_tail_finish_psi": [_p, _p, _d, _p, _p, _p, _p, _f, _l, _p, _l,
+                                   _i, _i, _p, _p, _i, _i, _p, _p, _p, _l, _p],
     "tike_lstsq_chunk_gradients": [_p, _p, _p, _p, _p, _i, _i, _p, _i, _p, _i,
                                    _f, _l, _p, _p, _p, _p, _p, _p, _p, _p, _f,
                                    _p, _i, _i, _i, _i, _i, _f, _f, _p],
diff --git a/tike_amd/_tuning.py b/tike_amd/_tuning.py
--- a/tike_amd/_tuning.py
+++ b/tike_amd/_tuning.py
@@ -16,6 +16,9 @@
 eigen_sums_gather = _flag("TIKE_EIGEN_SUMS_GATHER", True)
 stats_gather = _flag("TIKE_STATS_GATHER", False)
 fused_tail = _flag("TIKE_FUSED_TAIL", True)
+tail_prepare = _flag("TIKE_TAIL_PREPARE", True)
+tail_precond_norms = _flag("TIKE_TAIL_PRECOND_NORMS", True)
+tail_psi = _flag("TIKE_TAIL_PSI", True)
 precond_chunk = _int("TIKE_PRECOND_CHUNK", 512)
 multislice_slice_step = _flag("TIKE_MS_SLICE_STEP", True)
 multislice_first_stored = _flag("TIKE_MS_FIRST_STORED", True)
diff --git a/tike_amd/csrc/internal.h b/tike_amd/csrc/internal.h
--- a/tike_amd/csrc/internal.h
+++ b/tike_amd/csrc/internal.h
@@ -34,6 +34,23 @@
   else
     unsafeAtomicAdd(&k.costs[n], v);
 }
+__device__ __forceinline__ void tk_object_update_precond(
+    const float* __restrict__ acc, const cf* __restrict__ precond,
+    const float* __restrict__ pmax, float alpha, cf* __restrict__ upd_sum,
+    cf* __restrict__ upd_precond, float* __restrict__ combined, long npix, int b, int nb) {
+  const float am = alpha * pmax[0];
+  for (long i = b * 256L + threadIdx.x; i < npix; i += nb * 256L) {
+    const float re = acc[i], im = acc[npix + i];
+    const float p = (1.0f - alpha) * precond[i].x;
+    const float inv = 1.0f / sqrtf(p * p + am * am);
+    if (upd_sum) upd_sum[i] = mk(re, im);
+    if (upd_precond) upd_precond[i] = mk(re * inv, im * inv);
+    if (combined) {
+      combined[i] += re;
+      combined[npix + i] += im;
+    }
+  }
+}
 #endif
 int tk_cost_sink(float* costs, long nscan, int nslots, hipStream_t stream, TkCostSink* sink);
 int tk_cost_finish(const TkCostSink& sink, long nscan, hipStream_t stream);
diff --git a/tike_amd/csrc/lstsq.hip b/tike_amd/csrc/lstsq.hip
--- a/tike_amd/csrc/lstsq.hip
+++ b/tike_amd/csrc/lstsq.hip
@@ -832,14 +832,18 @@
   }
 }
 
-__global__ __launch_bounds__(256) void pass2_q_finish_kernel(const float* __restrict__ qtab,
-                                                             int slots, int nscan,
-                                                             float* __restrict__ q) {
-  const int n = blockIdx.x * 4 + (int)(threadIdx.x >> 6), k = threadIdx.x & 63;
+__device__ __forceinline__ void tk_q_finish(const float* __restrict__ qtab, int slots, int nscan,
+                                            float* __restrict__ q, int b) {
+  const int n = b * 4 + (int)(threadIdx.x >> 6), k = threadIdx.x & 63;
   if (n >= nscan) return;
   float a = k < slots ? qtab[(long)k * nscan + n] : 0.f;
   a = tk_wave_sum(a);
   if (k == 0) q[n] = a;
+}
+__global__ __launch_bounds__(256) void pass2_q_finish_kernel(const float* __restrict__ qtab,
+                                                             int slots, int nscan,
+                                                             float* __restrict__ q) {
+  tk_q_finish(qtab, slots, nscan, q, (int)blockIdx.x);
 }
 
 template <int N, int MW_, int MPW_>
@@ -868,8 +872,7 @@
   if (nscan == 0) return TK_OK;
   TK_CHECK_ARG(work && patches && (probe || !objproj));
   if (S > 8 || (det != 128 && det != 256 && det != 512)) return TK_ERR_UNSUPPORTED;
-  const bool qn = q != nullptr;
-  TK_CHECK_ARG(!qn || qtab);
+  const bool qn = qtab != nullptr;
   if (qn && (Stot != 0 || det > 256 || !objproj || !eigen_probe || !eigen_weights ||
              num_eigen < 1 || eigen_modes < 1))
     return TK_ERR_UNSUPPORTED;
@@ -968,7 +971,7 @@
 #undef TK_P2G_N
 #undef TK_P2G
   TK_LAUNCH_CHECK();
-  if (qn) {
+  if (q != nullptr) {
     hipLaunchKernelGGL(pass2_q_finish_kernel, dim3((nscan + 3) / 4), dim3(256), 0, stream,
                        qtab, det / 4, nscan, q);
     TK_LAUNCH_CHECK();
@@ -1012,7 +1015,7 @@
                                                 int nscan, int S, int det, float inv_scale,
                                                 float* qtab, float* q, void* stream) {
   TK_ENTER();
-  TK_CHECK_ARG(nscan == 0 || (qtab && q));
+  TK_CHECK_ARG(nscan == 0 || qtab);
   return launch_pass2_gradients(work, patches, probe, eigen_probe, eigen_weights, num_eigen,
                                 eigen_modes, objproj, chi0, m_probe_update, mpu_scale, nscan, S,
                                 det, inv_scale, nullptr, (hipStream_t)stream, 0, 0, qtab, q);
@@ -1636,18 +1639,43 @@
 }
 
 constexpr int TK_C0_PARTS = 64;
+__device__ __forceinline__ void tk_eigen_proj_offset(const cf* __restrict__ mpu0,
+                                                     const cf* __restrict__ E, long P,
+                                                     float* __restrict__ part, int b, float* red) {
+  float a = 0.f;
+  for (long p = b * 256L + threadIdx.x; p < P; p += 256L * TK_C0_PARTS) {
+    const cf m = mpu0[p], e = E[p];
+    a += m.x * e.x + m.y * e.y;
+  }
+  a = tk_block_sum256(a, red);
+  if (threadIdx.x == 0) part[b] = a;
+}
 __global__ __launch_bounds__(256) void eigen_proj_offset_kernel(const cf* __restrict__ mpu0,
                                                                 const cf* __restrict__ E,
                                                                 long P,
                                                                 float* __restrict__ part) {
   __shared__ float red[4];
-  float a = 0.f;
-  for (long p = blockIdx.x * 256L + threadIdx.x; p < P; p += 256L * TK_C0_PARTS) {
-    const cf m = mpu0[p], e = E[p];
-    a += m.x * e.x + m.y * e.y;
-  }
-  a = tk_block_sum256(a, red);
-  if (threadIdx.x == 0) part[blockIdx.x] = a;
+  tk_eigen_proj_offset(mpu0, E, P, part, (int)blockIdx.x, red);
+}
+
+__global__ __launch_bounds__(256) void tail_prepare1_kernel(
+    const float* __restrict__ qtab, int slots, int nscan, float* __restrict__ q,
+    const cf* __restrict__ mpu0, const cf* __restrict__ E, long P, float* __restrict__ part,
+    float* __restrict__ arena, long len, int nq) {
+  __shared__ float red[4];
+  int b = (int)blockIdx.x;
+  if (b < TK_C0_PARTS) {
+    tk_eigen_proj_offset(mpu0, E, P, part, b, red);
+    return;
+  }
+  b -= TK_C0_PARTS;
+  if (b < nq) {
+    tk_q_finish(qtab, slots, nscan, q, b);
+    return;
+  }
+  b -= nq;
+  const long nz = (long)gridDim.x - TK_C0_PARTS - nq;
+  for (long i = b * 256L + threadIdx.x; i < len; i += nz * 256L) arena[i] = 0.f;
 }
 
 __global__ __launch_bounds__(256) void eigen_pixel_update1_kernel(
@@ -2049,33 +2077,81 @@
   }
 }
 
+__device__ __forceinline__ void tk_eigen_norm_sums1(const cf* __restrict__ E,
+                                                    const cf* __restrict__ update, int npix,
+                                                    float* __restrict__ nacc,
+                                                    float* __restrict__ part, int b, int nb,
+                                                    float* red) {
+  float uu = 0.f, ee = 0.f, eu = 0.f;
+  for (int i = b * 256 + threadIdx.x; i < npix; i += nb * 256) {
+    const cf e = E[i], u = update[i];
+    uu += norm2(u);
+    ee += norm2(e);
+    eu += e.x * u.x + e.y * u.y;
+  }
+  uu = tk_block_sum256(uu, red);
+  ee = tk_block_sum256(ee, red);
+  eu = tk_block_sum256(eu, red);
+  if (threadIdx.x == 0) {
+    if (part != nullptr) {
+      part[3 * b] = uu;
+      part[3 * b + 1] = ee;
+      part[3 * b + 2] = eu;
+    } else {
+      unsafeAtomicAdd(&nacc[0], uu);
+      unsafeAtomicAdd(&nacc[1], ee);
+      unsafeAtomicAdd(&nacc[2], eu);
+    }
+  }
+}
 __global__ __launch_bounds__(256) void eigen_norm_sums1_kernel(const cf* __restrict__ E,
                                                                const cf* __restrict__ update,
                                                                int npix, float* __restrict__ nacc,
                                                                float* __restrict__ part) {
   __shared__ float red[4];
-  float uu = 0.f, ee = 0.f, eu = 0.f;
-  for (int i = blockIdx.x * 256 + threadIdx.x; i < npix; i += gridDim.x * 256) {
-    const cf e = E[i], u = update[i];
-    uu += norm2(u);
-    ee += norm2(e);
-    eu += e.x * u.x + e.y * u.y;
-  }
-  uu = tk_block_sum256(uu, red);
-  ee = tk_block_sum256(ee, red);
-  eu = tk_block_sum256(eu, red);
-  if (threadIdx.x == 0) {
-    if (part != nullptr) {
-      part[3 * blockIdx.x] = uu;
-      part[3 * blockIdx.x + 1] = ee;
-      part[3 * blockIdx.x + 2] = eu;
-    } else {
-      unsafeAtomicAdd(&nacc[0], uu);
-      unsafeAtomicAdd(&nacc[1], ee);
-      unsafeAtomicAdd(&nacc[2], eu);
-    }
-  }
-}
+  tk_eigen_norm_sums1(E, update, npix, nacc, part, (int)blockIdx.x, (int)gridDim.x, red);
+}
+
+__global__ __launch_bounds__(256) void object_precond_eigen_norms1_kernel(
+    const float* __restrict__ acc, const cf* __restrict__ precond, const float* __restrict__ pmax,
+    float alpha, cf* __restrict__ upd_precond, float* __restrict__ combined, long npix_obj,
+    const cf* __restrict__ E, const cf* __restrict__ update, int npix, float* __restrict__ nacc,
+    int nnorm) {
+  __shared__ float red[4];
+  const int b = (int)blockIdx.x;
+  if (b < nnorm)
+    tk_eigen_norm_sums1(E, update, npix, nacc, nullptr, b, nnorm, red);
+  else
+    tk_object_update_precond(acc, precond, pmax, alpha, nullptr, upd_precond, combined, npix_obj,
+                             b - nnorm, (int)gridDim.x - nnorm);
+}
+
+extern "C" int tike_object_precond_eigen_norms1(const float* acc, const void* precond,
+                                                const float* pmax, float alpha,
+                                                void* upd_precond, float* combined, long npix_obj,
+                                                const void* eigen0, const void* update, int npix,
+                                                float* nacc, void* stream) {
+  TK_ENTER();
+  TK_CHECK_ARG(npix_obj >= 1 && npix >= 1);
+  TK_CHECK_ARG(acc && precond && pmax && upd_precond && eigen0 && update && nacc);
+  if (tk_deterministic()) return TK_ERR_UNSUPPORTED;
+  const int nnorm = npix >= 256 * 64 ? 64 : (npix + 255) / 256;
+  const int nobj = tk_grid((npix_obj + 255) / 256, 8);
+  hipLaunchKernelGGL(object_precond_eigen_norms1_kernel, dim3(nnorm + nobj), dim3(256), 0,
+                     (hipStream_t)stream, acc, (const cf*)precond, pmax, alpha, (cf*)upd_precond,
+                     combined, npix_obj, (const cf*)eigen0, (const cf*)update, npix, nacc, nnorm);
+  TK_LAUNCH_CHECK();
+  return TK_OK;
+}
+
+constexpr int TK_STATS_NACC_GIVEN = 1, TK_STATS_ZEROED = 2;
+static int step_stats_eigen1(const void* chi, const float* scan,
+                             const void* object_update_precond, const void* probe,
+                             const void* eigen_probe, const float* eigen_weights,
+                             int eigen_modes, const void* m_probe_update, const void* patches,
+                             const void* update, float* nacc, double count, float beta_eigen,
+                             float* stats, float* sums5, int nscan, int S, int chi_modes, int pw,
+                             int H, int W, int flags, void* stream);
 
 extern "C" int tike_lstsq_step_stats_eigen1(const void* chi, const float* scan,
                                             const void* object_update_precond, const void* probe,
@@ -2086,6 +2162,35 @@
                                             float* sums5, int nscan, int S, int chi_modes,
                                             int pw, int H, int W, void* stream) {
   TK_ENTER();
+  return step_stats_eigen1(chi, scan, object_update_precond, probe, eigen_probe, eigen_weights,
+                           eigen_modes, m_probe_update, patches, update, nacc, count, beta_eigen,
+                           stats, sums5, nscan, S, chi_modes, pw, H, W, 0, stream);
+}
+
+extern "C" int tike_lstsq_step_stats_eigen1f(const void* chi, const float* scan,
+                                             const void* object_update_precond,
+                                             const void* probe, const void* eigen_probe,
+                                             const float* eigen_weights, int eigen_modes,
+                                             const void* m_probe_update, const void* patches,
+                                             const void* update, float* nacc, double count,
+                                             float beta_eigen, float* stats, float* sums5,
+                                             int nscan, int S, int chi_modes, int pw, int H,
+                                             int W, int flags, void* stream) {
+  TK_ENTER();
+  TK_CHECK_ARG((flags & ~(TK_STATS_NACC_GIVEN | TK_STATS_ZEROED)) == 0);
+  if (tk_deterministic() && flags != 0) return TK_ERR_UNSUPPORTED;
+  return step_stats_eigen1(chi, scan, object_update_precond, probe, eigen_probe, eigen_weights,
+                           eigen_modes, m_probe_update, patches, update, nacc, count, beta_eigen,
+                           stats, sums5, nscan, S, chi_modes, pw, H, W, flags, stream);
+}
+
+static int step_stats_eigen1(const void* chi, const float* scan,
+                             const void* object_update_precond, const void* probe,
+                             const void* eigen_probe, const float* eigen_weights,
+                             int eigen_modes, const void* m_probe_update, const void* patches,
+                             const void* update, float* nacc, double count, float beta_eigen,
+                             float* stats, float* sums5, int nscan, int S, int chi_modes, int pw,
+                             int H, int W, int flags, void* stream) {
   TK_CHECK_ARG(nscan >= 0 && S >= 1 && chi_modes >= 1 && pw >= 1 && H >= 1 && W >= 1 &&
                eigen_modes >= 1 && count > 0);
   TK_CHECK_ARG(probe && eigen_probe && eigen_weights && m_probe_update && update && nacc);
@@ -2098,24 +2203,26 @@
   if (!((pw % 256 == 0 || 256 % pw == 0) && pw % (nsplit * groups) == 0 &&
         (long)H * W < (1L << 28)))
     return TK_ERR_UNSUPPORTED;
-  int grid = P >= 256 * 64 ? 64 : (int)((P + 255) / 256);
-  float* part = nullptr;
-  if (tk_deterministic()) {
-    part = tk_det_scratch(sizeof(float) * 3 * (size_t)grid);
-    if (part == nullptr) grid = 1;
-  }
-  hipLaunchKernelGGL(eigen_norm_sums1_kernel, dim3(grid), dim3(256), 0, (hipStream_t)stream,
-                     (const cf*)eigen_probe, (const cf*)update, (int)P, nacc, part);
-  TK_LAUNCH_CHECK();
-  if (part != nullptr) {
-    int rc = tk_ordered_sum(nacc, part, 3, grid, true, (hipStream_t)stream);
-    if (rc) return rc;
+  if (!(flags & TK_STATS_NACC_GIVEN)) {
+    int grid = P >= 256 * 64 ? 64 : (int)((P + 255) / 256);
+    float* part = nullptr;
+    if (tk_deterministic()) {
+      part = tk_det_scratch(sizeof(float) * 3 * (size_t)grid);
+      if (part == nullptr) grid = 1;
+    }
+    hipLaunchKernelGGL(eigen_norm_sums1_kernel, dim3(grid), dim3(256), 0, (hipStream_t)stream,
+                       (const cf*)eigen_probe, (const cf*)update, (int)P, nacc, part);
+    TK_LAUNCH_CHECK();
+    if (part != nullptr) {
+      int rc = tk_ordered_sum(nacc, part, 3, grid, true, (hipStream_t)stream);
+      if (rc) return rc;
+    }
   }
   if (nscan == 0) return TK_OK;
   TK_CHECK_ARG(chi && scan && object_update_precond && patches && stats && sums5);
   const TkProbe pr = tk_make_probe(probe, 0, eigen_probe, eigen_weights, 1, eigen_modes, S, pw,
                                    nullptr);
-  if (nsplit > 1) {
+  if (nsplit > 1 && !(flags & TK_STATS_ZEROED)) {
     hipError_t e = hipMemsetAsync(stats, 0, sizeof(float) * 8 * (size_t)nscan, (hipStream_t)stream);
     if (e == hipSuccess)
       e = hipMemsetAsync(sums5, 0, sizeof(float) * 5 * (size_t)nscan, (hipStream_t)stream);
@@ -2229,6 +2336,30 @@
   return TK_OK;
 }
 
+static int eigen_pixel_update1q(const void* patches, const void* chi0, const void* mpu0,
+                                const void* eigen0, const float* q, const float* weights_c,
+                                long weights_row, const float* norm, void* update, int nscan,
+                                int pw, int chi_modes, const void* psi, const float* scan, int H,
+                                int W, float* c0part, float* eproj_out, bool form_c0,
+                                void* stream);
+
+extern "C" int tike_lstsq_tail_prepare1(const float* qtab, int slots, int nscan, float* q,
+                                        const void* mpu0, const void* eigen0, int npix,
+                                        float* c0part, float* arena, long arena_len,
+                                        void* stream) {
+  TK_ENTER();
+  TK_CHECK_ARG(nscan >= 0 && slots >= 1 && slots <= 64 && npix >= 1 && arena_len >= 0);
+  TK_CHECK_ARG(mpu0 && eigen0 && c0part && (arena || arena_len == 0));
+  TK_CHECK_ARG(nscan == 0 || (qtab && q));
+  const int nq = (nscan + 3) / 4;
+  const int nz = arena_len == 0 ? 0 : tk_grid((arena_len + 2047) / 2048, 1);
+  hipLaunchKernelGGL(tail_prepare1_kernel, dim3(TK_C0_PARTS + nq + nz), dim3(256), 0,
+                     (hipStream_t)stream, qtab, slots, nscan, q, (const cf*)mpu0,
+                     (const cf*)eigen0, (long)npix, c0part, arena, arena_len, nq);
+  TK_LAUNCH_CHECK();
+  return TK_OK;
+}
+
 extern "C" int tike_eigen_pixel_update1q(const void* patches, const void* chi0,
                                          const void* mpu0, const void* eigen0, const float* q,
                                          const float* weights_c, long weights_row,
@@ -2237,13 +2368,38 @@
                                          int H, int W, float* c0part, float* eproj_out,
                                          void* stream) {
   TK_ENTER();
+  return eigen_pixel_update1q(patches, chi0, mpu0, eigen0, q, weights_c, weights_row, norm,
+                              update, nscan, pw, chi_modes, psi, scan, H, W, c0part, eproj_out,
+                              true, stream);
+}
+
+extern "C" int tike_eigen_pixel_update1p(const void* patches, const void* chi0,
+                                         const void* mpu0, const void* eigen0, const float* q,
+                                         const float* weights_c, long weights_row,
+                                         const float* norm, void* update, int nscan, int pw,
+                                         int chi_modes, const void* psi, const float* scan,
+                                         int H, int W, const float* c0part, float* eproj_out,
+                                         void* stream) {
+  TK_ENTER();
+  return eigen_pixel_update1q(patches, chi0, mpu0, eigen0, q, weights_c, weights_row, norm,
+                              update, nscan, pw, chi_modes, psi, scan, H, W, (float*)c0part,
+                              eproj_out, false, stream);
+}
+
+static int eigen_pixel_update1q(const void* patches, const void* chi0, const void* mpu0,
+                                const void* eigen0, const float* q, const float* weights_c,
+                                long weights_row, const float* norm, void* update, int nscan,
+                                int pw, int chi_modes, const void* psi, const float* scan, int H,
+                                int W, float* c0part, float* eproj_out, bool form_c0,
+                                void* stream) {
   TK_CHECK_ARG(nscan >= 0 && pw >= 1 && chi_modes >= 1 && weights_row >= 1);
   if (nscan == 0) return TK_OK;
   TK_CHECK_ARG(!psi || (scan && H >= 1 && W >= 1));
   TK_CHECK_ARG(patches && chi0 && mpu0 && eigen0 && q && weights_c && norm && update && c0part);
   const long P = (long)pw * pw;
-  hipLaunchKernelGGL(eigen_proj_offset_kernel, dim3(TK_C0_PARTS), dim3(256), 0,
-                     (hipStream_t)stream, (const cf*)mpu0, (const cf*)eigen0, P, c0part);
+  if (form_c0)
+    hipLaunchKernelGGL(eigen_proj_offset_kernel, dim3(TK_C0_PARTS), dim3(256), 0,
+                       (hipStream_t)stream, (const cf*)mpu0, (const cf*)eigen0, P, c0part);
   float* part = nullptr;
   const int chunk = probe_chunk(nscan, 2 * P, &part);
   dim3 grid((unsigned)((P + 255) / 256) + 1, (unsigned)((nscan + chunk - 1) / chunk));
diff --git a/tike_amd/csrc/solver.hip b/tike_amd/csrc/solver.hip
--- a/tike_amd/csrc/solver.hip
+++ b/tike_amd/csrc/solver.hip
@@ -5,18 +5,8 @@
     const float* __restrict__ acc, const cf* __restrict__ precond,
     const float* __restrict__ pmax, float alpha, cf* __restrict__ upd_sum,
     cf* __restrict__ upd_precond, float* __restrict__ combined, long npix) {
-  const float am = alpha * pmax[0];
-  for (long i = blockIdx.x * 256L + threadIdx.x; i < npix; i += gridDim.x * 256L) {
-    const float re = acc[i], im = acc[npix + i];
-    const float p = (1.0f - alpha) * precond[i].x;
-    const float inv = 1.0f / sqrtf(p * p + am * am);
-    if (upd_sum) upd_sum[i] = mk(re, im);
-    if (upd_precond) upd_precond[i] = mk(re * inv, im * inv);
-    if (combined) {
-      combined[i] += re;
-      combined[npix + i] += im;
-    }
-  }
+  tk_object_update_precond(acc, precond, pmax, alpha, upd_sum, upd_precond, combined, npix,
+                           (int)blockIdx.x, (int)gridDim.x);
 }
 
 extern "C" int tike_object_update_precond(const float* acc, const void* precond,
@@ -486,7 +476,8 @@
     float* __restrict__ steps, cf* __restrict__ probe, cf* __restrict__ combined,
     const cf* __restrict__ mpu, float inv_num_batch, long nprobe, float* __restrict__ weights,
     long row, int S, int m, const float* __restrict__ stats, const float* __restrict__ sums5,
-    int B, int npix) {
+    int B, int npix, const cf* __restrict__ psi, const cf* __restrict__ object_update,
+    cf* __restrict__ psi_next, long npsi) {
   const float bp = tail3[1] * inv_count;
   const long stride = (long)gridDim.x * 256;
   const long i0 = blockIdx.x * 256L + threadIdx.x;
@@ -504,6 +495,13 @@
       if (combined) combined[i] = combined[i] + d * inv_num_batch;
     }
   }
+  if (psi_next != nullptr) {
+    const float bo = tail3[0] * inv_count;
+    for (long i = i0; i < npsi; i += stride) {
+      const cf o = object_update[i], x = psi[i];
+      psi_next[i] = mk(__fadd_rn(x.x, __fmul_rn(bo, o.x)), __fadd_rn(x.y, __fmul_rn(bo, o.y)));
+    }
+  }
   if (weights != nullptr) {
     const float inv_P = 1.0f / (float)npix;
     const float d_mean = sums5 ? tail3[2] * inv_count : 0.f;
@@ -517,29 +515,56 @@
   }
 }
 
+static int tail_finish(const float* tail3, const float* sums3, double count, float* steps,
+                       void* probe, void* combined, const void* mpu, float inv_num_batch,
+                       long nprobe, float* weights, long weights_row, int S, int m,
+                       const float* stats, const float* sums5, int B, int npix, const void* psi,
+                       const void* object_update, void* psi_next, long npsi, void* stream) {
+  TK_CHECK_ARG(tail3 && sums3 && steps && count > 0 && B >= 0 && nprobe >= 0 && npix >= 0);
+  TK_CHECK_ARG(!probe || mpu);
+  TK_CHECK_ARG(!psi_next || (psi && object_update && npsi >= 0 && psi_next != psi));
+  if (B == 0) {
+    weights = nullptr;
+    sums5 = nullptr;
+  }
+  TK_CHECK_ARG(!weights || (stats && weights_row >= 1 && S >= 1 && m >= 0 && m < S));
+  TK_CHECK_ARG(!sums5 || (weights && weights_row >= 2L * S && npix >= 1));
+  long work = 1;
+  if (probe && nprobe > work) work = nprobe;
+  if (weights && B > work) work = B;
+  if (psi_next && npsi > work) work = npsi;
+  hipLaunchKernelGGL(lstsq_tail_finish_kernel, dim3(tk_grid((work + 255) / 256, 8)), dim3(256), 0,
+                     (hipStream_t)stream, tail3, sums3, (float)(1.0 / count), steps, (cf*)probe,
+                     (cf*)combined, (const cf*)mpu, inv_num_batch, nprobe, weights, weights_row,
+                     S, m, stats, sums5, B, npix, (const cf*)psi, (const cf*)object_update,
+                     (cf*)psi_next, npsi);
+  TK_LAUNCH_CHECK();
+  return TK_OK;
+}
+
 extern "C" int tike_lstsq_tail_finish(const float* tail3, const float* sums3, double count,
                                       float* steps, void* probe, void* combined, const void* mpu,
                                       float inv_num_batch, long nprobe, float* weights,
                                       long weights_row, int S, int m, const float* stats,
                                       const float* sums5, int B, int npix, void* stream) {
   TK_ENTER();
-  TK_CHECK_ARG(tail3 && sums3 && steps && count > 0 && B >= 0 && nprobe >= 0 && npix >= 0);
-  TK_CHECK_ARG(!probe || mpu);
-  if (B == 0) {
-    weights = nullptr;
-    sums5 = nullptr;
-  }
-  TK_CHECK_ARG(!weights || (stats && weights_row >= 1 && S >= 1 && m >= 0 && m < S));
-  TK_CHECK_ARG(!sums5 || (weights && weights_row >= 2L * S && npix >= 1));
-  long work = 1;
-  if (probe && nprobe > work) work = nprobe;
-  if (weights && B > work) work = B;
-  hipLaunchKernelGGL(lstsq_tail_finish_kernel, dim3(tk_grid((work + 255) / 256, 8)), dim3(256), 0,
-                     (hipStream_t)stream, tail3, sums3, (float)(1.0 / count), steps, (cf*)probe,
-                     (cf*)combined, (const cf*)mpu, inv_num_batch, nprobe, weights, weights_row,
-                     S, m, stats, sums5, B, npix);
-  TK_LAUNCH_CHECK();
-  return TK_OK;
+  return tail_finish(tail3, sums3, count, steps, probe, combined, mpu, inv_num_batch, nprobe,
+                     weights, weights_row, S, m, stats, sums5, B, npix, nullptr, nullptr, nullptr,
+                     0, stream);
+}
+
+extern "C" int tike_lstsq_tail_finish_psi(const float* tail3, const float* sums3, double count,
+                                          float* steps, void* probe, void* combined,
+                                          const void* mpu, float inv_num_batch, long nprobe,
+                                          float* weights, long weights_row, int S, int m,
+                                          const float* stats, const float* sums5, int B, int npix,
+                                          const void* psi, const void* object_update,
+                                          void* psi_next, long npsi, void* stream) {
+  TK_ENTER();
+  TK_CHECK_ARG(psi && object_update && psi_next);
+  return tail_finish(tail3, sums3, count, steps, probe, combined, mpu, inv_num_batch, nprobe,
+                     weights, weights_row, S, m, stats, sums5, B, npix, psi, object_update,
+                     psi_next, npsi, stream);
 }
 
 static int chunk_body(
diff --git a/tike_amd/ptycho/solvers/_plan.py b/tike_amd/ptycho/solvers/_plan.py
--- a/tike_amd/ptycho/solvers/_plan.py
+++ b/tike_amd/ptycho/solvers/_plan.py
@@ -42,6 +42,8 @@
         "tike_lstsq_gradients": n * (S * P + 2 * P),
         "tike_scatter_patches": n * (P + box),
         "tike_lstsq_step_stats": n * (3 * P + 32),
+        "tike_eigen_pixel_update1p": n * (P + 8) + 3 * P,
+        "tike_lstsq_step_stats_eigen1f": n * (2 * P + 52) + 4 * P,
         "tike_gen_fwd_rows": n * (Tw + 2 * P + 8) + (S + C) * P,
         "tike_gen_cols_gradient": n * (2 * Tw + D),
         "tike_gen_inv_rows_gradients": n * (Tw + 3 * P) + S * P,
@@ -474,7 +476,8 @@
                     "inverse pass 2 + gradients (x poisson steps)")
             elif k.q is not None:
                 check(lib.tike_ifft2_pass2_gradients_eproj(
-                    *p2, A.ptr(b.qtab), A.ptr(k.q), st),
+                    *p2, A.ptr(b.qtab),
+                    None if getattr(k, "q_partials", False) else A.ptr(k.q), st),
                     "inverse pass 2 + gradients + eigen projection")
             else:
                 check(lib.tike_ifft2_pass2_gradients(*p2, st),
diff --git a/tike_amd/ptycho/solvers/lstsq.py b/tike_amd/ptycho/solvers/lstsq.py
--- a/tike_amd/ptycho/solvers/lstsq.py
+++ b/tike_amd/ptycho/solvers/lstsq.py
@@ -5,6 +5,7 @@
 import torch
 
 from ... import _arrays as A
+from ... import _lib
 from ... import _tuning
 from ... import linalg
 from ... import opt
@@ -237,21 +238,35 @@
             recover_psi=recover_psi, recover_probe=recover_probe,
             position_terms=position_terms, want_q=want_q)
 
-        object_update_precond = None
-        if recover_psi:
+        norm = (None if eigen_norms is None else
+                eigen_norms[batch_index:batch_index + 1])
+        fused = packed and _fused_tail_serves(
+            g, psi, eigen_probe, eigen_weights, comm, recover_psi=recover_psi,
+            recover_probe=recover_probe, norm=norm)
+        object_update_precond = precond = psi_next = None
+        if (fused and TAIL_PRECOND_NORMS and not _lib.DETERMINISTIC):
+            object_update_precond = torch.empty((1, H, W),
+                                                dtype=torch.complex64,
+                                                device=dev)
+            precond = (g["object_acc"], object_options.preconditioner, pmax,
+                       object_combined)
+        elif recover_psi:
             object_update_precond = _precondition_object_update(
                 g["object_acc"], object_options.preconditioner, pmax=pmax,
                 combined=object_combined)
+        if (fused and TAIL_PSI and not compact
+                and not object_options.use_adaptive_moment
+                and psi.dtype == torch.complex64 and psi.is_contiguous()):
+            psi_next = torch.empty_like(psi)
         if packed:
             bbeta_object, bbeta_probe = _packed_tail(
                 g, psi, scan, probe, eigen_probe, eigen_weights,
                 object_update_precond, lo, hi, comm, op=op,
                 num_batch=num_batch, recover_psi=recover_psi,
-                recover_probe=recover_probe,
-                norm=None if eigen_norms is None else
-                eigen_norms[batch_index:batch_index + 1],
+                recover_probe=recover_probe, norm=norm,
                 steps_row=steps[batch_index],
-                probe_combined_update=probe_combined_update)
+                probe_combined_update=probe_combined_update,
+                precond=precond, psi_next=psi_next)
         else:
             stats = _step_stats(g, psi, scan, probe, eigen_probe,
                                 object_update_precond, lo, hi, op=op)
@@ -267,7 +282,9 @@
                 out=steps[batch_index])
 
         if recover_psi:
-            if not compact:
+            if psi_next is not None:
+                psi = psi_next
+            elif not compact:
                 dpsi = bbeta_object * object_update_precond
                 if object_options.use_adaptive_moment:
                     dpsi, object_options.v, object_options.m = opt.momentum(
@@ -370,6 +387,23 @@
 the per-position part of the eigen projection, the eigen update runs before
 the step statistics, and the statistics and the eigen position sums are one
 pass over chi_n,0 and the patches (tike_lstsq_step_stats_eigen1)."""
+
+TAIL_PREPARE = _tuning.tail_prepare
+"""The fused tail: pass 2 leaves the partials of q, and one launch
+(tike_lstsq_tail_prepare1) adds them up, forms the partials of the eigen
+projection's offset and zeroes every accumulator of the tail -- two launches
+and three fills fewer.  (Deterministic mode and minibatches of several chunks
+keep the separate launches.)"""
+
+TAIL_PRECOND_NORMS = _tuning.tail_precond_norms
+"""The fused tail: the preconditioned object update and the norm sums of the
+eigen update as one launch after the eigen pixel update
+(tike_object_precond_eigen_norms1).  (Not in deterministic mode.)"""
+
+TAIL_PSI = _tuning.tail_psi
+"""The fused tail, object updated after every minibatch without momentum:
+psi + beta_object * object_update_precond formed by the launch that closes
+the minibatch (tike_lstsq_tail_finish_psi) instead of by two torch launches."""
 
 PACKED_TAIL = True
 """Tests set this to False to run the staged tail (one entry per step of the
@@ -446,6 +480,8 @@
         buf.qtab = _workspace(op).get("eigen_qtab", (min(plan.chunk, max(B, 1)),
                                                      det // 4),
                                       torch.float32, dev)
+    q_partials = bool(q is not None and TAIL_PREPARE and 0 < B <= plan.chunk
+                      and not _lib.DETERMINISTIC)
     c = SimpleNamespace(
         op=op, data=data, psi=psi, probe=probe, ep=ep, eigen_probe=eigen_probe,
         C=C, Sm=Sm, H=H, W=W, st=A.stream_ptr(), fwd_scale=fwd_scale,
@@ -468,7 +504,7 @@
             costs=buf.costs[rows],
             patches=None if buf.patches is None else buf.patches[rows],
             chi0=None if buf.chi0 is None else buf.chi0[rows],
-            q=None if q is None else q[rows])
+            q=None if q is None else q[rows], q_partials=q_partials)
         k.data_f32 = _once(lambda a=clo, b=chi_hi: A.data_f32(data, a, b))
         if k.w is not None and Sm > 0 and buf.unique is not None and (
                 not plan.no_farplane):
@@ -520,7 +556,8 @@
                 patches=None if buf.patches is None else buf.patches[:B],
                 object_acc=obj_acc, m_probe_update=m_probe_update,
                 costs=buf.costs[:B], count=count, local_count=B,
-                q=None if q is None else q[:B])
+                q=None if q is None else q[:B],
+                qtab=buf.qtab if q_partials else None)
 
 
 def all_mode_position_sums(op, objproj, psi, scan, probe, eigen_probe, weights,
@@ -600,7 +637,18 @@
 def _packed_tail(g, psi, scan, probe, eigen_probe, eigen_weights,
                  object_update_precond, lo, hi, comm, *, op, num_batch,
                  recover_psi, recover_probe, norm, steps_row,
-                 probe_combined_update):
+                 probe_combined_update, precond=None, psi_next=None):
+    if _fused_tail_serves(g, psi, eigen_probe, eigen_weights, comm,
+                          recover_psi=recover_psi, recover_probe=recover_probe,
+                          norm=norm):
+        return _fused_tail(g, psi, scan, probe, eigen_probe, eigen_weights,
+                           object_update_precond, lo, hi, op=op,
+                           num_batch=num_batch, recover_psi=recover_psi,
+                           recover_probe=recover_probe, norm=norm,
+                           steps_row=steps_row,
+                           probe_combined_update=probe_combined_update,
+                           precond=precond, psi_next=psi_next)
+    assert precond is None and psi_next is None
     B = hi - lo
     dev = psi.device
     st = A.stream_ptr()
@@ -623,15 +671,6 @@
     update = small[4:4 + 2 * P]
     nacc = small[4 + 2 * P:4 + 2 * P + 4]
     tail3 = small[4 + 2 * P + 4:4 + 2 * P + 7]
-    if (one and g.get("q") is not None and not comm.collective
-            and object_update_precond is not None and psi.shape[0] == 1):
-        return _fused_tail(g, psi, scan, probe, eigen_probe, eigen_weights,
-                           object_update_precond, lo, hi, op=op,
-                           num_batch=num_batch, recover_psi=recover_psi,
-                           recover_probe=recover_probe, norm=norm,
-                           steps_row=steps_row,
-                           probe_combined_update=probe_combined_update,
-                           sums3=sums3, update=update, nacc=nacc, tail3=tail3)
     stats = _step_stats(g, psi, scan, probe, eigen_probe,
                         object_update_precond, lo, hi, op=op)
     eps_total = float(np.float32(np.float32(1e-9) / P) * P)
@@ -688,10 +727,20 @@
             steps_row[3] if recover_probe else None)
 
 
+def _fused_tail_serves(g, psi, eigen_probe, eigen_weights, comm, *,
+                       recover_psi, recover_probe, norm):
+    return bool(g.get("q") is not None and recover_psi and recover_probe
+                and eigen_weights is not None and eigen_probe is not None
+                and eigen_probe.shape[-4] == 1 and eigen_probe.shape[-3] >= 1
+                and g["patches"] is not None
+                and g["m_probe_update"] is not None and norm is not None
+                and not comm.collective and psi.shape[0] == 1)
+
+
 def _fused_tail(g, psi, scan, probe, eigen_probe, eigen_weights,
                 object_update_precond, lo, hi, *, op, num_batch, recover_psi,
-                recover_probe, norm, steps_row, probe_combined_update, sums3,
-                update, nacc, tail3):
+                recover_probe, norm, steps_row, probe_combined_update,
+                precond=None, psi_next=None):
     B = hi - lo
     dev = psi.device
     st = A.stream_ptr()
@@ -706,42 +755,82 @@
     row = w_rows.shape[-2] * w_rows.shape[-1]
     E = eigen_probe[0, 0, 0]
     eps_total = float(np.float32(np.float32(1e-9) / P) * P)
-    stats = ws.get("stats", (max(B, 1), 8), torch.float32, dev)
-    sums5 = ws.get("eigen_sums5", (max(B, 1), 5), torch.float32, dev)
-    eproj = ws.get("eigen_proj", (max(B, 1),), torch.float32, dev)
+    prepare = g.get("qtab") is not None
+    nb = max(B, 1)
+    small = 4 + 2 * P + 8
+    if prepare:
+        arena = ws.get("tail_arena", (small + 13 * nb,), torch.float32, dev)
+        stats = arena[small:small + 8 * nb].view(nb, 8)
+        sums5 = arena[small + 8 * nb:].view(nb, 5)
+    else:
+        arena = ws.get("tail_small", (small,), torch.float32, dev)
+        arena.zero_()
+        stats = ws.get("stats", (nb, 8), torch.float32, dev)
+        sums5 = ws.get("eigen_sums5", (nb, 5), torch.float32, dev)
+    sums3 = arena[:3]
+    update = arena[4:4 + 2 * P]
+    nacc = arena[4 + 2 * P:4 + 2 * P + 4]
+    tail3 = arena[4 + 2 * P + 4:4 + 2 * P + 7]
+    eproj = ws.get("eigen_proj", (nb,), torch.float32, dev)
     c0part = ws.get("eigen_c0part", (64,), torch.float32, dev)
     g["eigen_proj"] = eproj[:B]
     gpsi = A.ptr(psi[0]) if EIGEN_PATCH_RECOMPUTE else None
     scan_b = A.ptr(scan[lo:hi])
+    if prepare:
+        check(
+            lib.tike_lstsq_tail_prepare1(
+                A.ptr(g["qtab"]), pw // 4, B, A.ptr(g["q"]),
+                A.ptr(mpu[0, 0, 0]), A.ptr(E), P, A.ptr(c0part), A.ptr(arena),
+                arena.numel(), st), "minibatch tail preparation")
+    pixel_update = (lib.tike_eigen_pixel_update1p if prepare else
+                    lib.tike_eigen_pixel_update1q)
     check(
-        lib.tike_eigen_pixel_update1q(
+        pixel_update(
             A.ptr(g["patches"]), A.ptr(g["chi0"]), A.ptr(mpu[0, 0, 0]),
             A.ptr(E), A.ptr(g["q"]), w_rows[:, 1, 0].data_ptr(), row,
             A.ptr(norm), A.ptr(update), B, pw, g["chi_modes"], gpsi, scan_b,
             H, W, A.ptr(c0part), A.ptr(eproj), st),
         "eigen pixel update")
     beta_eigen = min(0.1, 1.0 / num_batch)
-    check(
-        lib.tike_lstsq_step_stats_eigen1(
-            A.ptr(g["chi0"]), scan_b, A.ptr(object_update_precond),
-            A.ptr(probe), A.ptr(eigen_probe), A.ptr(g["w_old"]), Sm,
-            A.ptr(mpu), A.ptr(g["patches"]), A.ptr(update), A.ptr(nacc), count,
-            beta_eigen, A.ptr(stats), A.ptr(sums5), B, S, g["chi_modes"], pw,
-            H, W, st),
-        "step-size statistics + eigen position sums")
+    if precond is not None:
+        object_acc, preconditioner, pmax, combined = precond
+        check(
+            lib.tike_object_precond_eigen_norms1(
+                A.ptr(object_acc), A.ptr(preconditioner), A.ptr(pmax), 0.05,
+                A.ptr(object_update_precond), A.ptr(combined), H * W, A.ptr(E),
+                A.ptr(update), P, A.ptr(nacc), st),
+            "preconditioned object update + eigen norm sums")
+    stats_args = (
+        A.ptr(g["chi0"]), scan_b, A.ptr(object_update_precond), A.ptr(probe),
+        A.ptr(eigen_probe), A.ptr(g["w_old"]), Sm, A.ptr(mpu),
+        A.ptr(g["patches"]), A.ptr(update), A.ptr(nacc), count, beta_eigen,
+        A.ptr(stats), A.ptr(sums5), B, S, g["chi_modes"], pw, H, W)
+    flags = (1 if precond is not None else 0) | (2 if prepare else 0)
+    if flags:
+        check(lib.tike_lstsq_step_stats_eigen1f(*stats_args, flags, st),
+              "step-size statistics + eigen position sums")
+    else:
+        check(lib.tike_lstsq_step_stats_eigen1(*stats_args, st),
+              "step-size statistics + eigen position sums")
     check(
         lib.tike_lstsq_tail_solve1(
             A.ptr(E), A.ptr(update), P, A.ptr(nacc), beta_eigen, A.ptr(stats),
             A.ptr(g["costs"]), A.ptr(sums5), B, eps_total, count,
             int(recover_psi), int(recover_probe), A.ptr(sums3), A.ptr(tail3),
             st), "eigen probe + step solve")
-    check(
-        lib.tike_lstsq_tail_finish(
-            A.ptr(tail3), A.ptr(sums3), count, A.ptr(steps_row),
-            A.ptr(probe) if recover_probe else None,
-            A.ptr(probe_combined_update) if recover_probe else None,
-            A.ptr(mpu), 1.0 / num_batch, probe.numel(), w_rows.data_ptr(), row,
-            S, 0, A.ptr(stats), A.ptr(sums5), B, P, st), "minibatch tail")
+    finish_args = (
+        A.ptr(tail3), A.ptr(sums3), count, A.ptr(steps_row),
+        A.ptr(probe) if recover_probe else None,
+        A.ptr(probe_combined_update) if recover_probe else None,
+        A.ptr(mpu), 1.0 / num_batch, probe.numel(), w_rows.data_ptr(), row,
+        S, 0, A.ptr(stats), A.ptr(sums5), B, P)
+    if psi_next is not None:
+        check(
+            lib.tike_lstsq_tail_finish_psi(
+                *finish_args, A.ptr(psi), A.ptr(object_update_precond),
+                A.ptr(psi_next), psi.numel(), st), "minibatch tail + psi")
+    else:
+        check(lib.tike_lstsq_tail_finish(*finish_args, st), "minibatch tail")
     g["stats"] = stats[:B]
     g["sums5"] = sums5[:B]
     return (steps_row[2] if recover_psi else None,
```

New measurement: 219,500 patterns/s (median of 4 runs). No clear change (+0.2%).
